# hardcamls/video-coding

Measured on AMD Instinct MI355X. Metric: Mpixel/s decoded (1080p 4:2:0 batch), higher is better.
Workload: dtype int32

## Files before the change

### video-coding_amd/csrc/hvc_capi.hip

```cpp
#include <cmath>

#include "hvc_ctx.h"
#include "hvc_dct_fixed.h"

bool pin_to_ctx_cpus(const hvc_ctx *c) {
    if (!c->have_cpus) {
        if (c->have_default_cpus) (void)pthread_setaffinity_np(pthread_self(), sizeof(cpu_set_t), &c->default_cpus);
        return true;
    }
    return pthread_setaffinity_np(pthread_self(), sizeof(cpu_set_t), &c->cpus) == 0;
}

bool parse_cpulist(const char *s, cpu_set_t &set) {
    CPU_ZERO(&set);
    int n = 0;
    while (*s) {
        while (*s == ' ' || *s == '\n') s++;
        if (!*s) break;
        char *end = nullptr;
        const long a = std::strtol(s, &end, 10);
        if (end == s || a < 0) return false;
        long b = a;
        s = end;
        if (*s == '-') {
// ... 435 lines not shown
    c->profiling = enabled != 0;
    c->k_calls = 0;
    return HVC_OK;
} HVC_ABI_CATCH

int hvc_kernel_ms_history(hvc_ctx *c, float *ms, int n) try {
    if (!c || !ms || n < 1 || n > HVC_PROF_RING || (unsigned long long)n > c->k_calls) return HVC_E_INVALID_ARG;
    DeviceGuard g(c->device);
    for (int i = 0; i < n; i++) {
        int slot = (int)((c->k_calls - (unsigned long long)n + (unsigned long long)i) % HVC_PROF_RING);
        HIPCHK(c, hipEventSynchronize(c->k1[slot]));
        HIPCHK(c, hipEventElapsedTime(&ms[i], c->k0[slot], c->k1[slot]));
    }
    return HVC_OK;
} HVC_ABI_CATCH

int hvc_last_kernel_ms(hvc_ctx *c, float *ms) { return hvc_kernel_ms_history(c, ms, 1); }

int hvc_device_alloc(hvc_ctx *c, size_t bytes, void **out) try {
    if (!c || !out) return HVC_E_INVALID_ARG;
    DeviceGuard g(c->device);
    hipError_t e = hipMalloc(out, bytes ? bytes : 1);
    if (e != hipSuccess) {
        c->last_hip = (int)e;
        *out = nullptr;
        return HVC_E_OUT_OF_MEMORY;
    }
    return HVC_OK;
} HVC_ABI_CATCH

int hvc_device_free(hvc_ctx *c, void *p) try {
    if (!c) return HVC_E_INVALID_ARG;
    DeviceGuard g(c->device);
    HIPCHK(c, hipFree(p));
    return HVC_OK;
} HVC_ABI_CATCH

int hvc_memcpy_h2d(hvc_ctx *c, void *dst, const void *src, size_t bytes) try {
    if (!c || (!dst && bytes) || (!src && bytes)) return HVC_E_INVALID_ARG;
    DeviceGuard g(c->device);
    HIPCHK(c, hipMemcpyAsync(dst, src, bytes, hipMemcpyHostToDevice, c->stream));
    HIPCHK(c, hipStreamSynchronize(c->stream));
    return HVC_OK;
} HVC_ABI_CATCH

int hvc_memcpy_d2h(hvc_ctx *c, void *dst, const void *src, size_t bytes) try {
    if (!c || (!dst && bytes) || (!src && bytes)) return HVC_E_INVALID_ARG;
    DeviceGuard g(c->device);
    HIPCHK(c, hipMemcpyAsync(dst, src, bytes, hipMemcpyDeviceToHost, c->stream));
    HIPCHK(c, hipStreamSynchronize(c->stream));
    return HVC_OK;
} HVC_ABI_CATCH

int hvc_checksum_records(hvc_ctx *c, const void *data, size_t record_bytes, size_t record_stride, int n_records,
                         uint64_t *sums, int where) try {
    if (!c || !sums || n_records < 0 || (!data && n_records && record_bytes)) return HVC_E_INVALID_ARG;
    if (where != HVC_MEM_HOST && where != HVC_MEM_DEVICE) return HVC_E_INVALID_ARG;
    if (n_records == 0) return HVC_OK;
    if (n_records > 1 && record_stride < record_bytes) return HVC_E_INVALID_ARG;
    DeviceGuard g(c->device);
    if (!g.ok) return fail_hip(c, hipErrorInvalidDevice);
    const size_t sum_bytes = (size_t)n_records * sizeof(unsigned long long);
    const uint8_t *d = (const uint8_t *)data;
    int r;
    if (where == HVC_MEM_HOST) {
        const size_t bytes = (size_t)(n_records - 1) * record_stride + record_bytes;
        if ((r = grow(c, &c->d_in, &c->in_cap, bytes ? bytes : 1))) return r;
        if (bytes) HIPCHK(c, hipMemcpyAsync(c->d_in, data, bytes, hipMemcpyHostToDevice, c->stream));
        d = (const uint8_t *)c->d_in;
    }
    if ((r = grow(c, &c->d_sums, &c->sums_cap, sum_bytes))) return r;
    for (int r0 = 0; r0 < n_records; r0 += 65535)
        HIPCHK(c, hvc::launch_checksum(d + (size_t)r0 * record_stride, record_bytes, record_stride,
                                       n_records - r0 < 65535 ? n_records - r0 : 65535, (unsigned long long *)c->d_sums + r0, c->stream));
    HIPCHK(c, hipMemcpyAsync(sums, c->d_sums, sum_bytes, hipMemcpyDeviceToHost, c->stream));
    HIPCHK(c, hipStreamSynchronize(c->stream));
    return HVC_OK;
} HVC_ABI_CATCH

int hvc_last_wide_blocks(hvc_ctx *c, uint64_t *count) try {
    if (!c || !count) return HVC_E_INVALID_ARG;
    DeviceGuard g(c->device);
    unsigned long long v = 0;
    HIPCHK(c, hipMemcpyAsync(&v, c->d_fix_count + 2, sizeof v, hipMemcpyDeviceToHost, c->stream));
    HIPCHK(c, hipStreamSynchronize(c->stream));
    *count = c->wide_host >= 0 ? (uint64_t)c->wide_host : (uint64_t)v;
    return HVC_OK;
} HVC_ABI_CATCH

static void prepare_tables(const uint16_t *qtabs, int n_qtabs, int *qt, int *ethr, int *ethr_packed, unsigned *qpair) {
    for (int i = 0; i < n_qtabs * 64; i++) qt[i] = (int)qtabs[i];
    for (int t = 0; t < n_qtabs; t++) {
        unsigned qmax = 1;
        for (int i = 0; i < 64; i++) qmax = qtabs[t * 64 + i] > qmax ? qtabs[t * 64 + i] : qmax;
        unsigned long long m = HVC_GUARD_D / qmax;
        unsigned long long thr = m * m;
        ethr[t] = thr > 0x7ffffffeull ? 0x7ffffffe : (int)thr;
        m = HVC_GUARD_D_PACKED / qmax;
        thr = m * m;
        ethr_packed[t] = thr > 0x7ffffffeull ? 0x7ffffffe : (int)thr;
        static const int PAIRS[4][2] = {{HVC_PAIR_A_LO, HVC_PAIR_A_HI}, {HVC_PAIR_B_LO, HVC_PAIR_B_HI},
                                        {HVC_PAIR_C_LO, HVC_PAIR_C_HI}, {HVC_PAIR_Z_LO, HVC_PAIR_Z_HI}};
        for (int r = 0; r < 8; r++)
            for (int k = 0; k < 4; k++) {
                unsigned lo = qtabs[t * 64 + hvc::HVC_ZF[8 * r + PAIRS[k][0]]];
                unsigned hi = qtabs[t * 64 + hvc::HVC_ZF[8 * r + PAIRS[k][1]]];
                qpair[t * 32 + r * 4 + k] = (lo & 0xffffu) | (hi << 16);
            }
    }
}

static int upload_dcfix(hvc_ctx *c, const std::vector<unsigned> &ids, const std::vector<long long> &dcs, const unsigned **d_count,
                        const unsigned **d_ids, const long long **d_dcs) {
    const size_t n = ids.size();
    const size_t off_ids = 16, off_dcs = (off_ids + n * sizeof(unsigned) + 15) & ~(size_t)15;
    int r = grow(c, &c->d_dcfix, &c->dcfix_cap, off_dcs + n * sizeof(long long));
    if (r) return r;
    const unsigned cnt = (unsigned)n;
    char *base = (char *)c->d_dcfix;
    HIPCHK(c, hipMemcpyAsync(base, &cnt, sizeof cnt, hipMemcpyHostToDevice, c->stream));
    HIPCHK(c, hipMemcpyAsync(base + off_ids, ids.data(), n * sizeof(unsigned), hipMemcpyHostToDevice, c->stream));
    HIPCHK(c, hipMemcpyAsync(base + off_dcs, dcs.data(), n * sizeof(long long), hipMemcpyHostToDevice, c->stream));
    HIPCHK(c, hipStreamSynchronize(c->stream));
    *d_count = (const unsigned *)base;
    *d_ids = (const unsigned *)(base + off_ids);
    *d_dcs = (const long long *)(base + off_dcs);
    return HVC_OK;
}

template <class Params, class Geometry>
static void fill_geometry(Params &P, const Geometry &G, size_t coef_fs, size_t pixel_fs, int n_frames) {
    std::memset(&P, 0, sizeof P);
    P.coef_fs = coef_fs;
    P.pixel_fs = pixel_fs;
    P.n_frames = n_frames;
    P.n_comp = G.n_comp;
    P.tiles_per_frame = G.tiles_per_frame;
    for (int i = 0; i < G.n_comp; i++) P.comp[i] = G.comp[i];
}

static hvc::HardcamlParams hardcaml_params(const hvc::DecodeParams &P, const uint16_t *qtabs, int n_qtabs) {
    hvc::HardcamlParams H;
    fill_geometry(H, P, P.coef_fs, P.pixel_fs, P.n_frames);
    H.coefs = P.coefs;
    H.pixels = P.pixels;
    hvc::prepare_hardcaml_tables(qtabs, n_qtabs, H.qq);
    H.dc_plane = P.dc_plane;
    H.dc_fs = P.dc_fs;
    return H;
}

static int apply_wide_dc(hvc_ctx *c, const hvc::DecodeParams &P, const std::vector<WideFix> &wide, const uint16_t *qtabs,
                         int n_qtabs, int arith) {
    std::vector<unsigned> ids;
    std::vector<long long> dcs;
    for (const WideFix &w : wide) {
        for (int i = 0; i < P.n_comp; i++) {
            const hvc::CompK &K = P.comp[i];
            const size_t b0 = K.coef_off / 64;
            if (w.block < b0 || w.block >= b0 + (size_t)K.nblk) continue;
            const unsigned b = (unsigned)(w.block - b0);
            ids.push_back(((unsigned)w.frame * (unsigned)P.tiles_per_frame + (unsigned)K.tile0 + b / HVC_TILE) * HVC_TILE + b % HVC_TILE);
            dcs.push_back(w.dc);
            break;
        }
    }
    if (ids.empty()) return HVC_OK;
// ... 124 lines not shown

static int frames_per_launch_capped(int n_frames, unsigned long long blocks_per_frame, unsigned long long ids_per_frame) {
    int per = frames_per_launch(n_frames, blocks_per_frame);
    if (per > 65535) per = 65535;
    const unsigned long long by_ids = ids_per_frame ? ((1ull << 32) - 1) / ids_per_frame : (unsigned long long)per;
    if ((unsigned long long)per > by_ids) per = (int)by_ids;
    return per < 1 ? 1 : per;
}


static int reserve_fix_list(hvc_ctx *c, size_t entries) {
    if (entries <= c->fix_cap) return HVC_OK;
    void *p = c->d_fix_list;
    size_t cap = c->fix_cap * sizeof(unsigned);
    const int r = grow(c, &p, &cap, entries * sizeof(unsigned));
    c->d_fix_list = (unsigned *)p;
    c->fix_cap = cap / sizeof(unsigned);
    return r;
}

template <class Launch>
static hipError_t for_each_launch(int f0, int cnt, int per, hipEvent_t k0, hipEvent_t k1, Launch launch) {
    for (int f = f0; f < f0 + cnt; f += per) {
        const hipError_t e = launch(f, std::min(per, f0 + cnt - f), f == f0 ? k0 : nullptr, f + per >= f0 + cnt ? k1 : nullptr);
        if (e != hipSuccess) return e;
    }
    return hipSuccess;
}

template <class Up, class Run, class Down>
static int through_device(hvc_ctx *c, int n_frames, size_t in_bytes, size_t out_bytes, size_t coef_bytes, bool may_overlap, Up up, Run run,
                          Down down) {
    int r = grow(c, &c->d_in, &c->in_cap, in_bytes);
    if (r) return r;
    if ((r = grow(c, &c->d_out, &c->out_cap, out_bytes))) return r;
    if (may_overlap && n_frames >= 8 && coef_bytes >= ((size_t)64 << 20))
        return overlapped_parts(c, n_frames, up, [&](int, int f0, int cnt) { return run(f0, cnt); }, down);
    HIPCHK(c, up(0, n_frames));
    HIPCHK(c, run(0, n_frames));
    HIPCHK(c, down(0, n_frames, c->stream));
    HIPCHK(c, hipStreamSynchronize(c->stream));
    return HVC_OK;
}

static size_t tight_records(const hvc_component *comps, int n_comp, bool pixels, hvc_component *tight, int *blk0 = nullptr) {
    size_t at = 0;
    for (int i = 0; i < n_comp; i++) {
        tight[i] = comps[i];
        if (pixels) {
            tight[i].stride = (size_t)comps[i].blocks_w * 8;
            tight[i].plane_offset = at;
        } else {
            tight[i].coef_offset = at;
        }
        if (blk0) blk0[i] = (int)(at / 64);
        at += (size_t)comps[i].blocks_w * comps[i].blocks_h * 64;
    }
    return at;
}

int decode_frames_impl(hvc_ctx *c, const int16_t *coefs, size_t coef_fs, const uint16_t *qtabs, int n_qtabs,
                       const hvc_component *comps_in, int n_comp_in, int n_frames, uint8_t *pixels, size_t pixel_fs, int where,
                       const DecodeOpts &o) {
    if (!c || n_frames < 0) return HVC_E_INVALID_ARG;
    if (where != HVC_MEM_HOST && where != HVC_MEM_DEVICE) return HVC_E_INVALID_ARG;
    int r = check_qtabs(qtabs, n_qtabs, false);
    if (r) return r;
    hvc_component kept[HVC_MAX_COMP];
    int n_comp = 0;
    if ((r = drop_empty_components(comps_in, n_comp_in, kept, &n_comp))) return r;
    if (n_comp == 0) return HVC_OK;
    const hvc_component *const comps = kept;
    if (!coefs || !pixels) return HVC_E_INVALID_ARG;
    Layout L;
    r = make_layout(comps, n_comp, n_qtabs, L);
    if (r) return r;
    if (n_frames == 0) return HVC_OK;
    if (n_frames > 1 && (coef_fs < L.coef_span || pixel_fs < L.pixel_span)) return HVC_E_INVALID_ARG;
    if ((coef_fs & 7) || (pixel_fs & 7)) return HVC_E_ALIGNMENT;
    const unsigned long long ids_per_frame = (unsigned long long)L.tiles_per_frame * HVC_TILE;
    const int per = frames_per_launch_capped(n_frames, L.blocks_per_frame, ids_per_frame);
    const bool has_wide = o.wide && !o.wide->empty();
    if (has_wide && (unsigned long long)n_frames * ids_per_frame >= (1ull << 32)) return HVC_E_TOO_LARGE;
    DeviceGuard g(c->device);
    if (!g.ok) return fail_hip(c, hipErrorInvalidDevice);

    const bool twin = o.arith == HVC_ARITH_HARDCAML;
    if ((r = reserve_fix_list(c, twin ? 0 : (size_t)((unsigned long long)per * ids_per_frame)))) return r;

    hvc::DecodeParams P;
    fill_geometry(P, L, coef_fs, pixel_fs, n_frames);
    prepare_tables(qtabs, n_qtabs, P.qt, P.ethr, P.ethr_packed, P.qpair);
    wide_total_begin(c);
    fix_assign(c, P);

    bool wide_only = false;
    for (int i = 0; i < n_qtabs * 64; i++) wide_only |= qtabs[i] > 255;
    wide_only |= c->decode_kernel == 2;
    P.kernel_sel = (c->decode_kernel == 1 || c->decode_kernel == 3) ? c->decode_kernel : 0;
    if (wide_only) c->wide_host = (long long)((unsigned long long)n_frames * L.blocks_per_frame);
    if (twin) c->wide_host = 0;
    auto launch = [&](hvc::DecodeParams &Q, hipEvent_t k0, hipEvent_t k1) -> hipError_t {
        if (twin) return hvc::launch_hardcaml(hardcaml_params(Q, qtabs, n_qtabs), c->stream, k0, k1);
        if (wide_only) return hvc::launch_decode_wide_only(Q, c->stream, k0, k1);
        fix_assign(c, Q);
        const hipError_t e = hvc::launch_decode(Q, c->stream, k0, k1);
        if (e == hipSuccess) fix_commit(c);
        else fix_reset(c);
        return e;
    };
    auto launch_range = [&](const int16_t *d_coefs, uint8_t *d_pixels, int f0, int cnt, hipEvent_t k0, hipEvent_t k1) {
        return for_each_launch(f0, cnt, per, k0, k1, [&](int f, int n, hipEvent_t e0, hipEvent_t e1) {
            hvc::DecodeParams Pk = P;
            Pk.n_frames = n;
            Pk.coefs = d_coefs + (size_t)f * coef_fs;
            Pk.pixels = d_pixels + (size_t)f * pixel_fs;
            if (o.dc_plane) Pk.dc_plane = o.dc_plane + (size_t)f * o.dc_fs;
            return launch(Pk, e0, e1);
        });
    };

    if (where == HVC_MEM_DEVICE) {
        if (((uintptr_t)coefs & 15) || ((uintptr_t)pixels & 7)) return HVC_E_ALIGNMENT;
        if (o.dc_plane && P.kernel_sel != 0 && !twin) return HVC_E_INVALID_ARG;
        P.coefs = coefs;
        P.pixels = pixels;
        P.dc_plane = o.dc_plane;
        P.dc_fs = o.dc_fs;
        const int slot = (int)(c->k_calls % HVC_PROF_RING);
        HIPCHK(c, launch_range(coefs, pixels, 0, n_frames, o.profile ? c->k0[slot] : nullptr, o.profile ? c->k1[slot] : nullptr));
        if (o.profile) c->k_calls++;
        if (has_wide) return apply_wide_dc(c, P, *o.wide, qtabs, n_qtabs, o.arith);
        return HVC_OK;
    }
    if (o.dc_plane || has_wide) return HVC_E_INVALID_ARG;

    const size_t cbytes = ((size_t)(n_frames - 1) * coef_fs + L.coef_span) * sizeof(int16_t);
    const size_t pbytes = (size_t)(n_frames - 1) * pixel_fs + L.pixel_span;
    const RecordRun run = pixel_run(comps, n_comp);
    return through_device(
        c, n_frames, cbytes, pbytes, cbytes, run.len != 0,
        [&](int f0, int cnt) {
            return hipMemcpyAsync((int16_t *)c->d_in + (size_t)f0 * coef_fs, coefs + (size_t)f0 * coef_fs,
                                  ((size_t)(cnt - 1) * coef_fs + L.coef_span) * sizeof(int16_t), hipMemcpyHostToDevice, c->stream);
        },
        [&](int f0, int cnt) { return launch_range((const int16_t *)c->d_in, (uint8_t *)c->d_out, f0, cnt, nullptr, nullptr); },
        [&](int f0, int cnt, hipStream_t st) {
            return download_pixels(comps, n_comp, run, f0, cnt, pixel_fs, (const uint8_t *)c->d_out, pixels, st);
        });
}

int hvc_decode_frames(hvc_ctx *c, const int16_t *coefs, size_t coef_fs, const uint16_t *qtabs, int n_qtabs,
                      const hvc_component *comps, int n_comp, int n_frames, uint8_t *pixels, size_t pixel_fs,
                      int where) try {
    return decode_frames_impl(c, coefs, coef_fs, qtabs, n_qtabs, comps, n_comp, n_frames, pixels, pixel_fs, where, DecodeOpts(c));
} HVC_ABI_CATCH

int hvc_decode_frames_mixed(hvc_ctx *c, const int16_t *coefs, const size_t *coef_offsets, const hvc_jpeg_info *infos, int n_frames,
                            uint8_t *pixels, const size_t *pixel_offsets, int where) try {
    return decode_frames_mixed_impl(c, coefs, coef_offsets, infos, n_frames, pixels, pixel_offsets, where);
} HVC_ABI_CATCH

int decode_frames_scaled_impl(hvc_ctx *c, const int16_t *coefs, size_t coef_fs, const uint16_t *qtabs, int n_qtabs,
                              const hvc_component *comps_in, int n_comp_in, int n_frames, int scale_denom, uint8_t *pixels,
                              size_t pixel_fs, int where, const DecodeOpts &o) {
    const int N = scaled_side(scale_denom);
    if (!c || !N) return HVC_E_INVALID_ARG;
    if (N == 8) return decode_frames_impl(c, coefs, coef_fs, qtabs, n_qtabs, comps_in, n_comp_in, n_frames, pixels, pixel_fs, where, o);
    if (o.arith != HVC_ARITH_MODEL) return HVC_E_INVALID_ARG;
    if (n_frames < 0 || (where != HVC_MEM_HOST && where != HVC_MEM_DEVICE)) return HVC_E_INVALID_ARG;
    int r = check_qtabs(qtabs, n_qtabs, false);
    if (r) return r;
    hvc_component kept[HVC_MAX_COMP];
    int n_comp = 0;
    if ((r = drop_empty_components(comps_in, n_comp_in, kept, &n_comp))) return r;
    if (n_comp == 0) return HVC_OK;
    const hvc_component *const comps = kept;
    if (!coefs || !pixels) return HVC_E_INVALID_ARG;
    Layout L;
    if ((r = make_layout(comps, n_comp, n_qtabs, L, N))) return r;
    if (n_frames == 0) return HVC_OK;
    if (n_frames > 1 && (coef_fs < L.coef_span || pixel_fs < L.pixel_span)) return HVC_E_INVALID_ARG;
    if (coef_fs & 7) return HVC_E_ALIGNMENT;
    const int per = frames_per_launch_capped(n_frames, L.blocks_per_frame, (unsigned long long)L.tiles_per_frame * HVC_TILE);
    DeviceGuard g(c->device);
    if (!g.ok) return fail_hip(c, hipErrorInvalidDevice);

    hvc::DecodeParams P;
    fill_geometry(P, L, coef_fs, pixel_fs, n_frames);
    for (int i = 0; i < n_qtabs * 64; i++) P.qt[i] = (int)qtabs[i];
    P.wide_total = reinterpret_cast<unsigned long long *>(c->d_fix_count + 2);
    wide_total_begin(c);
    bool rows_on_dwords = ((n_frames > 1 ? pixel_fs : 0) & 3) == 0;
    for (int i = 0; i < n_comp; i++) rows_on_dwords &= ((comps[i].plane_offset | comps[i].stride) & 3) == 0;

    auto launch_range = [&](const int16_t *d_coefs, uint8_t *d_pixels, int f0, int cnt, hipEvent_t k0, hipEvent_t k1) {
        const bool dwords = rows_on_dwords && ((uintptr_t)d_pixels & 3) == 0;
        return for_each_launch(f0, cnt, per, k0, k1, [&](int f, int n, hipEvent_t e0, hipEvent_t e1) {
            hvc::DecodeParams Pk = P;
            Pk.n_frames = n;
            Pk.coefs = d_coefs + (size_t)f * coef_fs;
            Pk.pixels = d_pixels + (size_t)f * pixel_fs;
            Pk.dc_plane = o.dc_plane ? o.dc_plane + (size_t)f * o.dc_fs : nullptr;
            Pk.dc_fs = o.dc_fs;
            return hvc::launch_decode_scaled(Pk, N, dwords, c->stream, e0, e1);
        });
    };

    if (where == HVC_MEM_DEVICE) {
        if ((uintptr_t)coefs & 15) return HVC_E_ALIGNMENT;
        HIPCHK(c, hipMemsetAsync(P.wide_total, 0, sizeof *P.wide_total, c->stream));
        const int slot = (int)(c->k_calls % HVC_PROF_RING);
        HIPCHK(c, launch_range(coefs, pixels, 0, n_frames, o.profile ? c->k0[slot] : nullptr, o.profile ? c->k1[slot] : nullptr));
        if (o.profile) c->k_calls++;
        return HVC_OK;
    }
    if (o.dc_plane) return HVC_E_INVALID_ARG;

    const size_t cbytes = ((size_t)(n_frames - 1) * coef_fs + L.coef_span) * sizeof(int16_t);
    const size_t pbytes = (size_t)(n_frames - 1) * pixel_fs + L.pixel_span;
    return through_device(
        c, n_frames, cbytes, pbytes, cbytes, false,
        [&](int f0, int cnt) {
            const hipError_t e = hipMemsetAsync(P.wide_total, 0, sizeof *P.wide_total, c->stream);
            if (e != hipSuccess) return e;
            return hipMemcpyAsync((int16_t *)c->d_in + (size_t)f0 * coef_fs, coefs + (size_t)f0 * coef_fs,
                                  ((size_t)(cnt - 1) * coef_fs + L.coef_span) * sizeof(int16_t), hipMemcpyHostToDevice, c->stream);
        },
        [&](int f0, int cnt) { return launch_range((const int16_t *)c->d_in, (uint8_t *)c->d_out, f0, cnt, nullptr, nullptr); },
        [&](int f0, int cnt, hipStream_t st) {
            for (int f = f0; f < f0 + cnt; f++)
                for (int i = 0; i < n_comp; i++) {
                    const hvc_component &k = comps[i];
                    const size_t off = (size_t)f * pixel_fs + k.plane_offset;
                    const hipError_t e = hipMemcpy2DAsync(pixels + off, k.stride, (const uint8_t *)c->d_out + off, k.stride,
                                                          (size_t)k.blocks_w * N, (size_t)k.blocks_h * N, hipMemcpyDeviceToHost, st);
                    if (e != hipSuccess) return e;
                }
            return hipSuccess;
        });
}

int hvc_decode_frames_scaled(hvc_ctx *c, const int16_t *coefs, size_t coef_fs, const uint16_t *qtabs, int n_qtabs,
                             const hvc_component *comps, int n_comp, int n_frames, int scale_denom, uint8_t *pixels, size_t pixel_fs,
                             int where) try {
    return decode_frames_scaled_impl(c, coefs, coef_fs, qtabs, n_qtabs, comps, n_comp, n_frames, scale_denom, pixels, pixel_fs, where,
                                     DecodeOpts(c));
} HVC_ABI_CATCH

int hvc_decode_frames_rgb(hvc_ctx *c, const int16_t *coefs, size_t coef_fs, const uint16_t *qtabs, int n_qtabs, const hvc_component *comps,
                          int n_comp, int sampling, int n_frames, int width, int height, uint8_t *rgb, size_t rgb_row_stride,
                          size_t rgb_frame_stride, int layout, int where) try {
    RgbImage im;
    bool nothing = false;
    if (!coefs || !qtabs || !comps || !rgb) return HVC_E_INVALID_ARG;
    int r = rgb_check_args(c, sampling, width, height, n_frames, layout, where, rgb_row_stride, rgb_frame_stride, im, nothing);
    if (r) return r;
    if (n_comp != (sampling == HVC_YUV_400 ? 1 : 3)) return HVC_E_INVALID_ARG;
    if ((r = check_qtabs(qtabs, n_qtabs, false))) return r;
    if (nothing) return HVC_OK;
    int cw, ch;
    rgb_chroma_window(sampling, width, height, cw, ch);
    size_t coef_span = 0;
    for (int k = 0; k < n_comp; k++) {
        if (comps[k].blocks_w < 1 || comps[k].blocks_h < 1) return HVC_E_INVALID_ARG;
        if ((k ? cw : width) > 8 * comps[k].blocks_w || (k ? ch : height) > 8 * comps[k].blocks_h) return HVC_E_INVALID_ARG;
        coef_span = std::max(coef_span, comps[k].coef_offset + (size_t)comps[k].blocks_w * comps[k].blocks_h * 64);
    }
    hvc_component tight[HVC_MAX_COMP];
    const size_t px_fs = tight_records(comps, n_comp, true, tight);
    if (n_frames > 1 && coef_fs < coef_span) return HVC_E_INVALID_ARG;
    if (coef_fs & 7) return HVC_E_ALIGNMENT;
    if (where == HVC_MEM_DEVICE && ((uintptr_t)coefs & 15)) return HVC_E_ALIGNMENT;
    DeviceGuard g(c->device);
// ... 68 lines not shown
    int blk0[HVC_MAX_COMP];
    const size_t px_fs = tight_records(kept, n_comp, true, tight, blk0), blocks = px_fs / 64;
    Layout L;
    if ((r = make_layout(tight, n_comp, n_qtabs, L))) return r;
    if (n_frames > 1 && (coef_fs < L.coef_span || diff_fs < blocks)) return HVC_E_INVALID_ARG;
    if (coef_fs & 7) return HVC_E_ALIGNMENT;
    if (where == HVC_MEM_DEVICE && ((uintptr_t)coefs & 15)) return HVC_E_ALIGNMENT;
    DeviceGuard g(c->device);
    if (!g.ok) return fail_hip(c, hipErrorInvalidDevice);
    DecodeOpts model(c);
    model.arith = HVC_ARITH_MODEL;
    model.profile = false;
    return divergence_chunks(
        c, (const uint8_t *)coefs, coef_fs * sizeof(int16_t), L.coef_span * sizeof(int16_t), px_fs, n_frames, max_diff, diff_fs, blocks, where,
        [&](const uint8_t *d_in, int cnt) {
            return decode_frames_impl(c, (const int16_t *)d_in, coef_fs, qtabs, n_qtabs, tight, n_comp, cnt, (uint8_t *)c->d_div_px, px_fs,
                                      HVC_MEM_DEVICE, model);
        },
        [&](const uint8_t *d_in, int cnt, uint8_t *d_diff) {
            hvc::DecodeParams P;
            fill_geometry(P, L, coef_fs, px_fs, cnt);
            P.coefs = (const int16_t *)d_in;
            P.pixels = (uint8_t *)c->d_div_px;
            hvc::HardcamlParams H = hardcaml_params(P, qtabs, n_qtabs);
            H.diff = d_diff;
            H.diff_fs = diff_fs;
            for (int i = 0; i < n_comp; i++) H.blk0[i] = blk0[i];
            return hvc::launch_hardcaml(H, c->stream);
        });
} HVC_ABI_CATCH

int decode_frames_yuv444_impl(hvc_ctx *c, const int16_t *coefs, size_t coef_fs, const uint16_t *qtabs, int n_qtabs,
                              const hvc_component *comps, int n_comp, int n_frames, int width, int height, uint8_t *frames,
                              size_t frame_stride, int where, const DecodeOpts &o) {
    if (!c || !coefs || !frames || !comps || n_frames < 0) return HVC_E_INVALID_ARG;
    if (o.arith != HVC_ARITH_MODEL) return HVC_E_INVALID_ARG;
    if (where != HVC_MEM_HOST && where != HVC_MEM_DEVICE) return HVC_E_INVALID_ARG;
    int r = check_qtabs(qtabs, n_qtabs, false);
    if (r) return r;
    if (n_comp != 3 || width < 2 || height < 2 || (width & 1) || (height & 1)) return HVC_E_INVALID_ARG;
    if (width > 65535 || height > 65535) return HVC_E_TOO_LARGE;
    Layout L;
    hvc_component geo[3];
    for (int i = 0; i < 3; i++) {
        geo[i] = comps[i];
        geo[i].plane_offset = 0;
        geo[i].stride = comps[i].blocks_w > 0 ? (size_t)comps[i].blocks_w * 8 : 0;
    }
    r = make_layout(geo, n_comp, n_qtabs, L);
    if (r) return r;
    const int aw[3] = {width, width / 2, width / 2}, ah[3] = {height, height / 2, height / 2};
    for (int i = 0; i < 3; i++)
        if (comps[i].blocks_w * 8 < aw[i] || comps[i].blocks_h * 8 < ah[i]) return HVC_E_INVALID_ARG;
    const size_t plane_bytes = (size_t)width * (size_t)height, out_span = 3 * plane_bytes;
    if (n_frames == 0) return HVC_OK;
    if (n_frames > 1 && (coef_fs < L.coef_span || frame_stride < out_span)) return HVC_E_INVALID_ARG;
    if (coef_fs & 7) return HVC_E_ALIGNMENT;

    hvc::Decode444Params P;
    std::memset(&P, 0, sizeof P);
    P.coef_fs = coef_fs;
    P.out_fs = frame_stride;
    P.n_frames = n_frames;
    P.width = width;
    P.height = height;
    for (int i = 0; i < 3; i++) {
        hvc::Plane444K &K = P.pl[i];
        K.bw = comps[i].blocks_w;
        K.cbw = (aw[i] + 7) / 8;
        K.cbh = (ah[i] + 7) / 8;
        K.aw = aw[i];
        K.ah = ah[i];
        K.qtab = comps[i].qtab;
        K.coef_off = comps[i].coef_offset;
        K.out_off = (size_t)i * plane_bytes;
    }
    if ((unsigned long long)P.pl[0].cbw * P.pl[0].cbw * P.pl[0].cbh >= (1ull << 32)) return HVC_E_TOO_LARGE;
    const bool aligned = width % 16 == 0 && frame_stride % 16 == 0 && (where == HVC_MEM_HOST || (uintptr_t)frames % 16 == 0);
    hvc::plan_decode_444(P, aligned);
    const unsigned long long ids_per_frame = (unsigned long long)P.tiles_per_frame * HVC_TILE * P.nw;
    const int per = frames_per_launch_capped(n_frames, L.blocks_per_frame, ids_per_frame);
    const bool has_wide = o.wide && !o.wide->empty();
    if (has_wide && (unsigned long long)n_frames * ids_per_frame >= (1ull << 32)) return HVC_E_TOO_LARGE;
    const unsigned long long ids = (unsigned long long)per * ids_per_frame;
    DeviceGuard g(c->device);
    if (!g.ok) return fail_hip(c, hipErrorInvalidDevice);
    int ethr_unused[HVC_MAX_QTABS];
    prepare_tables(qtabs, n_qtabs, P.qt, ethr_unused, P.ethr_packed, P.qpair);
    bool wide_only = c->decode_kernel == 2;
    for (int i = 0; i < n_qtabs * 64; i++) wide_only |= qtabs[i] > 255;
    const int split = (aligned && !wide_only && c->decode_kernel == 0 && height % 8 == 0 && P.pl[0].cbw == P.pl[0].bw) ? fused444_mode() : 0;
    const size_t luma_ids = split ? (size_t)per * (size_t)((P.pl[0].cbw * P.pl[0].cbh + HVC_TILE - 1) / HVC_TILE) * HVC_TILE : 0;
    if ((r = reserve_fix_list(c, luma_ids + (size_t)ids))) return r;
    P.fix_list = c->d_fix_list;
    wide_total_begin(c);
    if (split == 2 && !c->side_stream) {
        static const int prio_sel = [] { const char *v = std::getenv("HVC_444_SIDE_PRIO"); return v ? std::atoi(v) : 0; }();
        int least = 0, greatest = 0;
        HIPCHK(c, hipDeviceGetStreamPriorityRange(&least, &greatest));
        HIPCHK(c, hipStreamCreateWithPriority(&c->side_stream, hipStreamNonBlocking, prio_sel < 0 ? greatest : prio_sel > 0 ? least : 0));
        HIPCHK(c, hipEventCreateWithFlags(&c->ev_fork, hipEventDisableTiming));
        HIPCHK(c, hipEventCreateWithFlags(&c->ev_join, hipEventDisableTiming));
    }
    auto launch_split = [&](hvc::Decode444Params &Q, hipEvent_t k0, hipEvent_t k1) -> hipError_t {
        const hvc::Plane444K &K = Q.pl[0];
        hvc::DecodeParams Y;
        std::memset(&Y, 0, sizeof Y);
        Y.coefs = Q.coefs;
        Y.pixels = Q.out;
        Y.coef_fs = Q.coef_fs;
        Y.pixel_fs = Q.out_fs;
        Y.n_frames = Q.n_frames;
        Y.n_comp = 1;
        Y.comp[0].bw = K.cbw;
        Y.comp[0].bh = K.cbh;
        Y.comp[0].nblk = K.cbw * K.cbh;
        Y.comp[0].magic = K.cbw == 1 ? 0u : (unsigned)(((1ull << 32) + (unsigned)K.cbw - 1) / (unsigned)K.cbw);
        Y.comp[0].qtab = K.qtab;
        Y.comp[0].coef_off = K.coef_off;
        Y.comp[0].plane_off = K.out_off;
        Y.comp[0].stride = (size_t)Q.width;
        Y.tiles_per_frame = (Y.comp[0].nblk + HVC_TILE - 1) / HVC_TILE;
        prepare_tables(qtabs, n_qtabs, Y.qt, Y.ethr, Y.ethr_packed, Y.qpair);
        Y.dc_plane = Q.dc_plane;
        Y.dc_fs = Q.dc_fs;
        Y.fix_count = c->d_fix_count + 4 + c->fix_phase_l;
        Y.fix_count_next = c->d_fix_count + 4 + (c->fix_phase_l ^ 1);
        Y.fix_list = c->d_fix_list + (size_t)ids;
        Y.wide_total = reinterpret_cast<unsigned long long *>(c->d_fix_count + 2);
        fix_assign(c, Q);
        Q.tile0 = Q.y_tiles;
        hipStream_t ys = c->stream;
        hipError_t e = hipSuccess;
        if (k0) e = hipEventRecord(k0, c->stream);
        if (split == 2) {
            if (e == hipSuccess && !c->wide_total_started) e = hipMemsetAsync(Y.wide_total, 0, sizeof(unsigned long long), c->stream);
            Y.wide_first = Q.wide_first = 2;
            if (e == hipSuccess) e = hipEventRecord(c->ev_fork, c->stream);
            if (e == hipSuccess) e = hipStreamWaitEvent(c->side_stream, c->ev_fork, 0);
            ys = c->side_stream;
        } else {
            Y.wide_first = Q.wide_first;
            Q.wide_first = 0;
        }
        if (e == hipSuccess) e = hvc::launch_decode(Y, ys, nullptr, nullptr);
        if (e == hipSuccess) c->fix_phase_l ^= 1;
        if (e == hipSuccess) e = hvc::launch_decode_444(Q, false, c->stream, nullptr, nullptr);
        if (e == hipSuccess && split == 2) {
            e = hipEventRecord(c->ev_join, c->side_stream);
            if (e == hipSuccess) e = hipStreamWaitEvent(c->stream, c->ev_join, 0);
        }
        if (e == hipSuccess && k1) e = hipEventRecord(k1, c->stream);
        if (e == hipSuccess) fix_commit(c);
        else {
            if (c->side_stream) (void)hipStreamSynchronize(c->side_stream);
            fix_reset(c);
        }
        return e;
    };
    auto launch = [&](hvc::Decode444Params &Q, hipEvent_t k0, hipEvent_t k1) -> hipError_t {
        if (wide_only) {
            c->wide_host = (long long)n_frames * ((long long)P.pl[0].cbw * P.pl[0].cbh + 2ll * P.pl[1].cbw * P.pl[1].cbh);
            return hvc::launch_decode_444(Q, true, c->stream, k0, k1);
        }
        if (split) return launch_split(Q, k0, k1);
        fix_assign(c, Q);
        const hipError_t e = hvc::launch_decode_444(Q, false, c->stream, k0, k1);
        if (e == hipSuccess) fix_commit(c);
        else fix_reset(c);
        return e;
    };

    auto launch_range = [&](const int16_t *d_coefs, uint8_t *d_out, int f0, int cnt, hipEvent_t k0, hipEvent_t k1) {
        return for_each_launch(f0, cnt, per, k0, k1, [&](int f, int n, hipEvent_t e0, hipEvent_t e1) {
            hvc::Decode444Params Pk = P;
            Pk.n_frames = n;
            Pk.coefs = d_coefs + (size_t)f * coef_fs;
            Pk.out = d_out + (size_t)f * frame_stride;
            if (o.dc_plane) Pk.dc_plane = o.dc_plane + (size_t)f * o.dc_fs;
            return launch(Pk, e0, e1);
        });
    };

    if (where == HVC_MEM_HOST && (o.dc_plane || has_wide)) return HVC_E_INVALID_ARG;
    if (where == HVC_MEM_DEVICE) {
        if ((uintptr_t)coefs & 15) return HVC_E_ALIGNMENT;
        P.coefs = coefs;
        P.out = frames;
        P.dc_plane = o.dc_plane;
        P.dc_fs = o.dc_fs;
        const bool prof = o.profile && !wide_only;
        const int slot = (int)(c->k_calls % HVC_PROF_RING);
        HIPCHK(c, launch_range(coefs, frames, 0, n_frames, prof ? c->k0[slot] : nullptr, prof ? c->k1[slot] : nullptr));
        if (prof) c->k_calls++;
        if (has_wide) return apply_wide_dc_444(c, P, *o.wide);
        return HVC_OK;
    }
    const size_t cbytes = ((size_t)(n_frames - 1) * coef_fs + L.coef_span) * sizeof(int16_t);
    const size_t obytes = (size_t)(n_frames - 1) * frame_stride + out_span;
    return through_device(
        c, n_frames, cbytes, obytes, cbytes, true,
        [&](int f0, int cnt) {
            return hipMemcpyAsync((int16_t *)c->d_in + (size_t)f0 * coef_fs, coefs + (size_t)f0 * coef_fs,
                                  ((size_t)(cnt - 1) * coef_fs + L.coef_span) * sizeof(int16_t), hipMemcpyHostToDevice, c->stream);
        },
        [&](int f0, int cnt) { return launch_range((const int16_t *)c->d_in, (uint8_t *)c->d_out, f0, cnt, nullptr, nullptr); },
        [&](int f0, int cnt, hipStream_t st) {
            return copy_run_d2h((const uint8_t *)c->d_out, frames, 0, out_span, frame_stride, f0, cnt, st);
        });
}

int hvc_decode_frames_yuv444(hvc_ctx *c, const int16_t *coefs, size_t coef_fs, const uint16_t *qtabs, int n_qtabs,
// ... 470 lines not shown
```

### video-coding_amd/csrc/hvc_capi_mixed.hip

```cpp
#include "hvc_ctx.h"
#include "hvc_mixed.h"

namespace {

struct ImageParts {
    size_t planes = 0, tables = 0, map = 0, total = 0;
};
ImageParts image_parts(const hvc::MixedPlan &plan) {
    ImageParts p;
    auto up = [](size_t v) { return (v + 15) & ~(size_t)15; };
    p.planes = 0;
    p.tables = up(plan.planes.size() * sizeof(hvc::MixedPlaneK));
    p.map = p.tables + up(plan.tables.size() * sizeof(hvc::MixedTableK));
    p.total = p.map + up(plan.map.size() * sizeof(unsigned));
    return p;
}

int upload_plan(hvc_ctx *c, const hvc::MixedPlan &plan, hvc::MixedParams &P) {
    const ImageParts ip = image_parts(plan);
    std::vector<unsigned char> img(ip.total, 0);
    std::memcpy(img.data() + ip.planes, plan.planes.data(), plan.planes.size() * sizeof(hvc::MixedPlaneK));
    std::memcpy(img.data() + ip.tables, plan.tables.data(), plan.tables.size() * sizeof(hvc::MixedTableK));
    std::memcpy(img.data() + ip.map, plan.map.data(), plan.map.size() * sizeof(unsigned));
    if (!c->ev_mixed) HIPCHK(c, hipEventCreateWithFlags(&c->ev_mixed, hipEventDisableTiming));
    const bool same = c->mixed_len == ip.total && c->h_mixed && !std::memcmp(c->h_mixed, img.data(), ip.total);
    if (!same) {
        c->mixed_len = 0;
        int r = grow(c, &c->d_mixed, &c->mixed_cap, ip.total);
        if (r) return r;
        if (ip.total > c->h_mixed_cap) {
            HIPCHK(c, hipStreamSynchronize(c->stream));
            if (c->h_mixed) (void)hipHostFree(c->h_mixed);
            c->h_mixed = nullptr;
            c->h_mixed_cap = 0;
            const size_t want = ip.total + ip.total / 4 + 4096;
            if (hipHostMalloc(&c->h_mixed, want, hipHostMallocDefault) != hipSuccess) {
                c->h_mixed = nullptr;
                return HVC_E_OUT_OF_MEMORY;
            }
            c->h_mixed_cap = want;
        } else {
            HIPCHK(c, wait_event(c->ev_mixed));
        }
        std::memcpy(c->h_mixed, img.data(), ip.total);
        HIPCHK(c, hipMemcpyAsync(c->d_mixed, c->h_mixed, ip.total, hipMemcpyHostToDevice, c->stream));
        HIPCHK(c, hipEventRecord(c->ev_mixed, c->stream));
        c->mixed_len = ip.total;
    }
    const unsigned char *d = (const unsigned char *)c->d_mixed;
    P.planes = reinterpret_cast<const hvc::MixedPlaneK *>(d + ip.planes);
    P.tables = reinterpret_cast<const hvc::MixedTableK *>(d + ip.tables);
    P.map = reinterpret_cast<const unsigned *>(d + ip.map);
    P.n_units = (unsigned)plan.map.size();
    return HVC_OK;
}

int reserve_mixed_fix_list(hvc_ctx *c, size_t entries) {
    if (entries <= c->fix_cap) return HVC_OK;
    void *p = c->d_fix_list;
    size_t cap = c->fix_cap * sizeof(unsigned);
    const int r = grow(c, &p, &cap, entries * sizeof(unsigned));
    c->d_fix_list = (unsigned *)p;
    c->fix_cap = cap / sizeof(unsigned);
    return r;
}

int mixed_launch_plan(hvc_ctx *c, const hvc::MixedPlan &plan, const int16_t *d_coefs, uint8_t *d_pixels, bool profile) {
    int r;
    if (plan.map.empty()) return HVC_OK;
    if (((uintptr_t)d_coefs & 15) || ((uintptr_t)d_pixels & 7)) return HVC_E_ALIGNMENT;
    if ((r = reserve_mixed_fix_list(c, plan.map.size() * HVC_MIXED_UNIT))) return r;
    hvc::MixedParams P;
    std::memset(&P, 0, sizeof P);
    if ((r = upload_plan(c, plan, P))) return r;
    P.coefs = d_coefs;
    P.pixels = d_pixels;
    P.all_wide = c->decode_kernel == 2;
    fix_assign(c, P);
    const int slot = (int)(c->k_calls % HVC_PROF_RING);
    const hipError_t e = hvc::launch_decode_mixed(P, c->stream, profile ? c->k0[slot] : nullptr, profile ? c->k1[slot] : nullptr);
    if (e != hipSuccess) {
        fix_reset(c);
        return fail_hip(c, e);
    }
    fix_commit(c);
    if (profile) c->k_calls++;
    return HVC_OK;
}

int mixed_launch(hvc_ctx *c, const int16_t *d_coefs, const size_t *coef_offsets, const hvc_jpeg_info *infos, const int *frames,
                 int n_list, uint8_t *d_pixels, const size_t *pixel_offsets, bool profile) {
    hvc::MixedPlan plan;
    const int r = hvc::mixed_plan_build(infos, coef_offsets, pixel_offsets, frames, n_list, plan);
    return r ? r : mixed_launch_plan(c, plan, d_coefs, d_pixels, profile);
}

void frame_spans(const hvc_jpeg_info &fi, size_t &coef_span, size_t &pixel_span) {
    coef_span = pixel_span = 0;
    for (int i = 0; i < fi.n_comp && i < 4; i++) {
        const hvc_component &k = fi.layout[i];
        if (k.blocks_w <= 0 || k.blocks_h <= 0) continue;
        coef_span = std::max(coef_span, k.coef_offset + (size_t)k.blocks_w * k.blocks_h * 64);
        pixel_span = std::max(pixel_span, k.plane_offset + ((size_t)k.blocks_h * 8 - 1) * k.stride + (size_t)k.blocks_w * 8);
    }
}

}

int decode_frames_mixed_impl(hvc_ctx *c, const int16_t *coefs, const size_t *coef_offsets, const hvc_jpeg_info *infos, int n_frames,
                             uint8_t *pixels, const size_t *pixel_offsets, int where) {
    if (!c || n_frames < 0 || (where != HVC_MEM_HOST && where != HVC_MEM_DEVICE)) return HVC_E_INVALID_ARG;
    if (c->arith != HVC_ARITH_MODEL) return HVC_E_INVALID_ARG;
    if (n_frames == 0) return HVC_OK;
    if (!infos || !coef_offsets || !pixel_offsets) return HVC_E_INVALID_ARG;
    DeviceGuard g(c->device);
    if (!g.ok) return fail_hip(c, hipErrorInvalidDevice);
    int r;
    {
        hvc::MixedPlan plan;
        if ((r = hvc::mixed_plan_build(infos, coef_offsets, pixel_offsets, nullptr, n_frames, plan))) return r;
        if (plan.map.empty()) return HVC_OK;
        if (!coefs || !pixels) return HVC_E_INVALID_ARG;
        if (where == HVC_MEM_DEVICE) {
            wide_total_begin(c);
            return mixed_launch_plan(c, plan, coefs, pixels, c->profiling);
        }
    }
    std::vector<size_t> d_coef((size_t)n_frames), d_pix((size_t)n_frames), cspan((size_t)n_frames);
    size_t ctot = 0, ptot = 0;
    for (int f = 0; f < n_frames; f++) {
        size_t ps;
        frame_spans(infos[f], cspan[(size_t)f], ps);
        d_coef[(size_t)f] = ctot;
        d_pix[(size_t)f] = ptot;
        ctot += (cspan[(size_t)f] + 63) & ~(size_t)63;
        ptot += (ps + 63) & ~(size_t)63;
    }
    if ((r = grow(c, &c->d_in, &c->in_cap, ctot * sizeof(int16_t)))) return r;
    if ((r = grow(c, &c->d_out, &c->out_cap, ptot))) return r;
    for (int f = 0; f < n_frames; f++)
        if (cspan[(size_t)f])
            HIPCHK(c, hipMemcpyAsync((int16_t *)c->d_in + d_coef[(size_t)f], coefs + coef_offsets[f], cspan[(size_t)f] * sizeof(int16_t),
                                     hipMemcpyHostToDevice, c->stream));
    wide_total_begin(c);
    if ((r = mixed_launch(c, (const int16_t *)c->d_in, d_coef.data(), infos, nullptr, n_frames, (uint8_t *)c->d_out, d_pix.data(), false))) {
        (void)hipStreamSynchronize(c->stream);
        return r;
    }
    for (int f = 0; f < n_frames; f++)
        for (int i = 0; i < infos[f].n_comp; i++) {
            const hvc_component &k = infos[f].layout[i];
            if (k.blocks_w <= 0 || k.blocks_h <= 0) continue;
            const size_t row = (size_t)k.blocks_w * 8, rows = (size_t)k.blocks_h * 8;
            uint8_t *dst = pixels + pixel_offsets[f] + k.plane_offset;
// ... 269 lines not shown
```

### video-coding_amd/csrc/hvc_ctx.h

```cpp
#ifndef HVC_CTX_H
#define HVC_CTX_H

#include <hip/hip_runtime.h>
#include <pthread.h>
#include <sched.h>

#include <algorithm>
#include <atomic>
#include <chrono>
#include <condition_variable>
#include <cstdio>
#include <cstdlib>
#include <cstring>
#include <mutex>
#include <new>
#include <thread>
#include <deque>
#include <functional>
#include <vector>

#include "../../include/hvc_jpeg.h"
#include "hvc_hdec.h"
#include "hvc_hardcaml.h"
#include "hvc_huff.h"
#include "hvc_kernels.h"
#include "hvc_pool.h"
#include "hvc_scaled_spec.h"

#define HVC_PROF_RING 64
#define HVC_FIX_WORDS 8

struct hvc_ctx {
    int device = -1;
    hipStream_t own_stream = nullptr;
    hipStream_t stream = nullptr;
    hipEvent_t ev0 = nullptr, ev1 = nullptr;
    hipEvent_t k0[HVC_PROF_RING] = {}, k1[HVC_PROF_RING] = {};
    unsigned long long k_calls = 0;
    bool profiling = false;
    bool honour_restart = false;
    int decode_kernel = 0;
    int arith = HVC_ARITH_MODEL;
    int enc_arith = HVC_ARITH_MODEL;
    int huff_tables = HVC_HUFF_DEFAULT;
    int restart_interval = 0;
    unsigned *d_fix_count = nullptr;
    int fix_phase_l = 0;
    hipStream_t side_stream = nullptr;
    hipEvent_t ev_fork = nullptr, ev_join = nullptr;
    bool wide_total_started = false;
    long long wide_host = -1;
    int fix_phase = 0;
    int fix_last = 0;
    unsigned *d_fix_list = nullptr;
    size_t fix_cap = 0;
    void *d_in = nullptr, *d_out = nullptr, *d_sums = nullptr, *d_aux = nullptr, *d_aux2 = nullptr;
    size_t in_cap = 0, out_cap = 0, sums_cap = 0, aux_cap = 0, aux2_cap = 0;
    void *d_div_px = nullptr, *d_div_in = nullptr, *d_div_out = nullptr;
    size_t div_px_cap = 0, div_in_cap = 0, div_out_cap = 0;
    void *d_dct_tab = nullptr, *d_dct_a = nullptr, *d_dct_b = nullptr;
    size_t dct_a_cap = 0, dct_b_cap = 0;
    int last_hip = 0;
    static constexpr int RING = 3;
    hipStream_t copy_stream = nullptr, down_stream = nullptr;
    hipStream_t rd_stream[3] = {};
    hipEvent_t ev_rd[3] = {};
    void *h_ring[RING] = {}, *d_ring[RING] = {}, *d_oring[RING] = {};
    size_t ring_bytes = 0, oring_bytes = 0;
    hipEvent_t ev_h2d[RING] = {}, ev_kern[RING] = {}, ev_t[4] = {};
    void *eh_in[RING] = {}, *ed_in[RING] = {}, *eh_out[RING] = {}, *ed_out[RING] = {};
    size_t e_in_bytes = 0, e_out_bytes = 0;
    hipEvent_t ev_up[RING] = {}, ev_down[RING] = {}, ev_et[RING][3] = {}, ev_gpu[RING] = {};
    void *ed_seg[RING] = {}, *ed_off[RING] = {}, *eh_off[RING] = {};
    size_t e_seg_bytes = 0, e_off_bytes = 0;
    void *eh_specs[RING] = {};
    size_t e_specs_bytes = 0;
    void *gp_h_ecs[RING] = {}, *gp_d_ecs[RING] = {}, *gp_h_meta[RING] = {}, *gp_d_meta[RING] = {};
    void *gp_h_ftabs[RING] = {}, *gp_d_ftabs[RING] = {};
    size_t gp_ecs_bytes = 0, gp_meta_bytes = 0, gp_ftabs_bytes = 0;
    void *gd_ecs = nullptr, *gd_meta = nullptr, *gd_state = nullptr, *gd_tables = nullptr, *gd_coefs = nullptr, *gd_dcd = nullptr;
    void *gd_h_ecs = nullptr;
    size_t gd_h_ecs_cap = 0;
    void *gd_fcnt = nullptr;
    size_t gd_fcnt_cap = 0;
    void *gd_ftabs = nullptr;
    size_t gd_ftabs_cap = 0;
    void *gd_dcv = nullptr;
    size_t gd_dcv_cap = 0;
    void *d_dcfix = nullptr;
    size_t dcfix_cap = 0;
    void *d_mixed = nullptr, *h_mixed = nullptr;
    size_t mixed_cap = 0, h_mixed_cap = 0, mixed_len = 0;
    hipEvent_t ev_mixed = nullptr;
    bool have_cpus = false;
    cpu_set_t cpus;
    char cpulist[256] = "";
    bool have_default_cpus = false;
    cpu_set_t default_cpus;
    hvc::WorkerPool pool;
    hvc::HdTables *gd_tables_host = nullptr;
    bool gd_tables_valid = false;
    int gd_tables_ncomp = 0;
    size_t gd_ecs_cap = 0, gd_meta_cap = 0, gd_state_cap = 0, gd_tables_cap = 0, gd_coefs_cap = 0, gd_dcd_cap = 0;
    unsigned *hd_tables = nullptr;
    void *hd_opt = nullptr;
    size_t hd_opt_cap = 0;
    void *hd_lens = nullptr, *hd_meta = nullptr, *hd_bitbuf = nullptr, *hd_ff = nullptr, *hd_out = nullptr;
    size_t hd_lens_cap = 0, hd_meta_cap = 0, hd_bitbuf_cap = 0, hd_ff_cap = 0, hd_out_cap = 0;
    void *hd_ivl = nullptr;
    size_t hd_ivl_cap = 0;
    struct Slot {
        void *d_in = nullptr, *d_out = nullptr;
        size_t in_cap = 0, out_cap = 0;
        hipEvent_t up0 = nullptr, up1 = nullptr, k0 = nullptr, k1 = nullptr, dn0 = nullptr, dn1 = nullptr;
        bool busy = false, has_down = false, timed = false;
        unsigned long long h2d_bytes = 0, d2h_bytes = 0;
    } slots[HVC_SLOTS];
};

#ifndef HVC_UPLOAD_RING_FLAGS
#define HVC_UPLOAD_RING_FLAGS hipHostMallocDefault
#endif

struct DeviceGuard {
    int prev = -1;
    bool ok = true;
    explicit DeviceGuard(int dev) {
        if (hipGetDevice(&prev) != hipSuccess) prev = -1;
        if (prev != dev) ok = hipSetDevice(dev) == hipSuccess;
    }
    ~DeviceGuard() {
        int cur = -1;
        if (prev >= 0 && hipGetDevice(&cur) == hipSuccess && cur != prev) (void)hipSetDevice(prev);
    }
};

inline int fail_hip(hvc_ctx *c, hipError_t e) {
    c->last_hip = (int)e;
    return HVC_E_HIP;
}
#define HIPCHK(c, call)                                 \
    do {                                                \
        hipError_t e_ = (call);                         \
        if (e_ != hipSuccess) return fail_hip((c), e_); \
    } while (0)

bool pin_to_ctx_cpus(const hvc_ctx *c);

inline int pool_ready(hvc_ctx *c, int n, int extra = 0) { return c->pool.ensure(n + extra); }

bool parse_cpulist(const char *s, cpu_set_t &set);

int grow(hvc_ctx *c, void **p, size_t *cap, size_t need);

template <class Params>
inline void fix_assign(const hvc_ctx *c, Params &P) {
    P.fix_count = c->d_fix_count + c->fix_phase;
    P.fix_count_next = c->d_fix_count + (c->fix_phase ^ 1);
    P.fix_list = c->d_fix_list;
    P.wide_total = reinterpret_cast<unsigned long long *>(c->d_fix_count + 2);
    P.wide_first = c->wide_total_started ? 0 : 1;
}
inline void fix_commit(hvc_ctx *c) {
    c->fix_last = c->fix_phase;
    c->fix_phase ^= 1;
    c->wide_total_started = true;
}
inline void wide_total_begin(hvc_ctx *c) {
    c->wide_total_started = false;
    c->wide_host = -1;
}
inline void fix_reset(hvc_ctx *c) {
    (void)hipMemsetAsync(c->d_fix_count, 0, HVC_FIX_WORDS * sizeof(unsigned), c->stream);
}

size_t launch_bytes_limit();
#ifndef HVC_444_MODE_DEFAULT
#define HVC_444_MODE_DEFAULT 0
#endif
int fused444_mode();
int frames_per_launch(int n_frames, unsigned long long blocks_per_frame);

struct Layout {
    hvc::CompK comp[HVC_MAX_COMP];
    int n_comp = 0, tiles_per_frame = 0;
    size_t coef_span = 0;
    size_t pixel_span = 0;
    unsigned long long blocks_per_frame = 0;
};
int make_layout(const hvc_component *comps, int n_comp, int n_qtabs, Layout &L, int n = 8);
int check_qtabs(const uint16_t *qtabs, int n_qtabs, bool divides);

int drop_empty_components(const hvc_component *comps, int n_comp, hvc_component *kept, int *n_kept);

struct RecordRun {
    size_t first = 0, len = 0;
};
RecordRun pixel_run(const hvc_component *comps, int n_comp);
RecordRun coef_run(const hvc_component *comps, int n_comp);
hipError_t download_pixels(const hvc_component *comps, int n_comp, const RecordRun &run, int f0, int cnt, size_t fs,
                           const uint8_t *d_base, uint8_t *h_base, hipStream_t st);
hipError_t download_coefs(const hvc_component *comps, int n_comp, const RecordRun &run, int f0, int cnt, size_t fs_bytes,
                          const uint8_t *d_base, uint8_t *h_base, hipStream_t st);

hipError_t wait_event(hipEvent_t e);

template <class Up, class Run, class Down>
inline int overlapped_parts(hvc_ctx *c, int n_frames, Up up, Run run, Down down) {
    constexpr int K = 4;
    if (!c->down_stream) HIPCHK(c, hipStreamCreateWithFlags(&c->down_stream, hipStreamNonBlocking));
    for (int i = 0; i < K; i++)
        if (!c->ev_t[i]) HIPCHK(c, hipEventCreate(&c->ev_t[i]));
    std::atomic<int> launched{0}, herr{0};
    auto part = [&](int k, int &f0, int &cnt) {
        f0 = (int)((long long)n_frames * k / K);
        cnt = (int)((long long)n_frames * (k + 1) / K) - f0;
    };
    int pr = pool_ready(c, 1);
    if (pr) return pr;
    hvc::PoolScope scope(c->pool, [&] { if (launched.load() < K) herr.store(herr.load() ? herr.load() : (int)hipErrorUnknown); });
    pr = c->pool.submit([&] {
        (void)pin_to_ctx_cpus(c);
        if (hipSetDevice(c->device) != hipSuccess) { herr.store((int)hipErrorInvalidDevice); return; }
        for (int k = 0; k < K; k++) {
            while (launched.load(std::memory_order_acquire) <= k && !herr.load()) std::this_thread::yield();
            if (herr.load()) return;
            int f0, cnt;
            part(k, f0, cnt);
            hipError_t e = hipStreamWaitEvent(c->down_stream, c->ev_t[k], 0);
            if (e == hipSuccess) e = down(f0, cnt, c->down_stream);
            if (e == hipSuccess) e = hipStreamSynchronize(c->down_stream);
            if (e != hipSuccess) { herr.store((int)e); return; }
        }
    }, 1);
    if (pr) return pr;
    hipError_t e = hipSuccess;
    for (int k = 0; k < K && e == hipSuccess && !herr.load(); k++) {
        int f0, cnt;
        part(k, f0, cnt);
        e = up(f0, cnt);
        if (e == hipSuccess) e = run(k, f0, cnt);
        if (e == hipSuccess) e = hipEventRecord(c->ev_t[k], c->stream);
        if (e == hipSuccess) launched.store(k + 1, std::memory_order_release);
// ... 132 lines not shown
```

### video-coding_amd/csrc/hvc_kernels.h

```cpp
#ifndef HVC_KERNELS_H
#define HVC_KERNELS_H

#include <hip/hip_runtime.h>
#include <cstdlib>
#include <stddef.h>
#include <stdint.h>

#define HVC_MAX_COMP 4
#define HVC_MAX_QTABS 4
#define HVC_GUARD_D ((1 << 17) - 1)
#define HVC_TILE 256

#include "hvc_idct_spec.h"

namespace hvc {

static const unsigned char HVC_ZF[64] = {
    0,  1,  5,  6,  14, 15, 27, 28, 2,  4,  7,  13, 16, 26, 29, 42, 3,  8,  12, 17, 25, 30,
    41, 43, 9,  11, 18, 24, 31, 40, 44, 53, 10, 19, 23, 32, 39, 45, 52, 54, 20, 22, 33, 38,
    46, 51, 55, 60, 21, 34, 37, 47, 50, 56, 59, 61, 35, 36, 48, 49, 57, 58, 62, 63};

struct CompK {
    int bw, bh;
    int nblk;
    int tile0;
    unsigned magic;
    int qtab;
    size_t coef_off;
    size_t plane_off;
    size_t stride;
};

struct DecodeParams {
    const int16_t *coefs;
    uint8_t *pixels;
    size_t coef_fs;
    size_t pixel_fs;
    int n_frames, n_comp, tiles_per_frame;
    int kernel_sel;
    CompK comp[HVC_MAX_COMP];
    int qt[HVC_MAX_QTABS * 64];
    int ethr[HVC_MAX_QTABS];
    unsigned qpair[HVC_MAX_QTABS * 32];
    int ethr_packed[HVC_MAX_QTABS];
    unsigned *fix_count;
    unsigned *fix_count_next;
    unsigned *fix_list;
    const int16_t *dc_plane;
    size_t dc_fs;
    unsigned long long *wide_total;
    int wide_first;
    int xcd_map;
    unsigned xcd_magic;
};

struct EncodeParams {
    const uint8_t *pixels;
    int16_t *coefs;
    size_t coef_fs, pixel_fs;
    int n_frames, n_comp, tiles_per_frame, xcd_map;
    unsigned xcd_magic, pad;
    CompK comp[HVC_MAX_COMP];
    float qrcp[HVC_MAX_QTABS * 64];
};

struct UpsampleParams {
    const uint8_t *src;
    uint8_t *dst;
    int cw, ch, n_planes, xcd_map;
    size_t src_stride, dst_stride, src_ps, dst_ps;
    unsigned xcd_magic, pad;
};

struct Plane444K {
    int bw;
    int cbw, cbh;
    int aw, ah;
    int qtab;
    size_t coef_off;
    size_t out_off;
};

#define HVC_444_TILE_BW 64
#define HVC_444_TILE_BH 4

struct Decode444Params {
    const int16_t *coefs;
    uint8_t *out;
    size_t coef_fs;
    size_t out_fs;
    int n_frames, tiles_per_frame;
    int width, height;
    int y_tiles;
    unsigned y_magic;
    int c_tiles_x, c_tiles_y;
    unsigned c_magic;
    int skip;
    int nw;
    int tile0;
    Plane444K pl[3];
    int qt[HVC_MAX_QTABS * 64];
    unsigned qpair[HVC_MAX_QTABS * 32];
    int ethr_packed[HVC_MAX_QTABS];
    unsigned *fix_count, *fix_count_next, *fix_list;
    const int16_t *dc_plane;
    size_t dc_fs;
    unsigned long long *wide_total;
    int wide_first;
    int xcd_map;
    unsigned xcd_magic;
};

inline int xcd_map_run(bool fused = false) {
    static const int run = [] { const char *v = getenv("HVC_XCD_RUN"); return v ? atoi(v) : -1; }();
    static const int run444 = [] { const char *v = getenv("HVC_XCD_RUN_444"); return v ? atoi(v) : -1; }();
    if (fused) return run444 >= 0 ? run444 : run >= 0 ? run : 64;
    return run >= 0 ? run : 16;
}
#ifdef __HIPCC__
__device__ __forceinline__ void xcd_work(int map, unsigned magic, unsigned &frame, unsigned &tile) {
    frame = blockIdx.y;
    tile = blockIdx.x;
    if (map > 0) {
        const unsigned per = gridDim.x, id = frame * per + tile, sh = (unsigned)map - 1u;
        const unsigned group = 8u << sh, total = per * gridDim.y;
        if (id < total - total % group) {
            const unsigned k = id >> 3;
            const unsigned lin = ((((k >> sh) << 3) + (id & 7u)) << sh) + (k & ((1u << sh) - 1u));
            frame = __umulhi(lin, magic);
            tile = lin - frame * per;
        }
    }
}
#endif
inline int xcd_map_for(unsigned per, unsigned n, unsigned &magic, bool fused = false) {
    magic = per > 1 ? (unsigned)(((1ull << 32) + per - 1) / per) : 0u;
    const int run = xcd_map_run(fused);
    if (run <= 0 || per <= 1 || (unsigned long long)per * n * per >= (1ull << 32)) return 0;
    int sh = 0;
    while ((1 << (sh + 1)) <= run) sh++;
    return sh + 1;
}

hipError_t launch_decode_444(const Decode444Params &P, bool wide_only, hipStream_t s, hipEvent_t k0 = nullptr,
                             hipEvent_t k1 = nullptr);
void plan_decode_444(Decode444Params &P, bool aligned);
hipError_t launch_decode(const DecodeParams &P, hipStream_t s, hipEvent_t k0 = nullptr, hipEvent_t k1 = nullptr);
hipError_t launch_decode_wide_only(const DecodeParams &P, hipStream_t s, hipEvent_t k0 = nullptr, hipEvent_t k1 = nullptr);
hipError_t launch_decode_dcfix(const DecodeParams &P, const unsigned *count, const unsigned *ids, const long long *dcs,
                               hipStream_t s);
hipError_t launch_decode_444_dcfix(const Decode444Params &P, const unsigned *count, const unsigned *ids, const long long *dcs,
                                   unsigned n_host, hipStream_t s);
hipError_t launch_encode(const EncodeParams &P, hipStream_t s, hipEvent_t k0 = nullptr, hipEvent_t k1 = nullptr);
hipError_t launch_upsample420(const UpsampleParams &P, hipStream_t s);
hipError_t launch_abs_error(const EncodeParams &P, const uint8_t *recon, uint8_t *error, hipStream_t s);
#define HVC_CHECKSUM_MUL 0x9E3779B97F4A7C15ull
hipError_t launch_checksum(const uint8_t *data, size_t record_bytes, size_t record_stride, int n_records,
                           unsigned long long *sums, hipStream_t s);

}
#endif
```

### video-coding_amd/csrc/hvc_kernels.hip

```cpp

#include <hip/hip_runtime.h>
#include <stdint.h>
#include <stdlib.h>
#include <string.h>

#include "hvc_idct_spec.h"
#include "hvc_kernels.h"

#ifndef HVC_FAST_LB
#define HVC_FAST_LB HVC_TILE
#endif

namespace hvc {

__device__ constexpr int ZI[64] = {
    0,  1,  8,  16, 9,  2,  3,  10, 17, 24, 32, 25, 18, 11, 4,  5,
    12, 19, 26, 33, 40, 48, 41, 34, 27, 20, 13, 6,  7,  14, 21, 28,
    35, 42, 49, 56, 57, 50, 43, 36, 29, 22, 15, 23, 30, 37, 44, 51,
    58, 59, 52, 45, 38, 31, 39, 46, 53, 60, 61, 54, 47, 55, 62, 63};
__device__ constexpr int ZF[64] = {
    0,  1,  5,  6,  14, 15, 27, 28, 2,  4,  7,  13, 16, 26, 29, 42,
    3,  8,  12, 17, 25, 30, 41, 43, 9,  11, 18, 24, 31, 40, 44, 53,
    10, 19, 23, 32, 39, 45, 52, 54, 20, 22, 33, 38, 46, 51, 55, 60,
    21, 34, 37, 47, 50, 56, 59, 61, 35, 36, 48, 49, 57, 58, 62, 63};
// ... 147 lines not shown
    size_t coef_idx;
    size_t pix_idx;
    size_t stride;
    int qtab;
    size_t plane_coef_idx;
    int tile_b0;
    int nblk;
};

template <class Params>
__device__ __forceinline__ bool locate(const Params &P, int frame, int tile, int lane, BlockRef &br) {
    int c = 0;
#pragma unroll
    for (int i = 1; i < HVC_MAX_COMP; i++)
        if (i < P.n_comp && tile >= P.comp[i].tile0) c = i;
    const CompK &K = P.comp[c];
    int b = (tile - K.tile0) * HVC_TILE + lane;
    bool active = b < K.nblk;
    b = active ? b : K.nblk - 1;
    unsigned by = K.bw == 1 ? (unsigned)b : __umulhi((unsigned)b, K.magic);
    unsigned bx = (unsigned)b - by * (unsigned)K.bw;
    br.coef_idx = (size_t)frame * P.coef_fs + K.coef_off + (size_t)b * 64;
    br.pix_idx = (size_t)frame * P.pixel_fs + K.plane_off + (size_t)by * 8 * K.stride + (size_t)bx * 8;
    br.stride = K.stride;
    br.qtab = K.qtab;
    br.plane_coef_idx = (size_t)frame * P.coef_fs + K.coef_off;
    br.tile_b0 = (tile - K.tile0) * HVC_TILE;
    br.nblk = K.nblk;
    return active;
}

__global__ __launch_bounds__(HVC_FAST_LB) void k_decode_fast(DecodeParams P) {
    BlockRef br;
    const int lane = threadIdx.x;
    const bool active = locate(P, blockIdx.y, blockIdx.x, lane, br);

    const uint4 *src = reinterpret_cast<const uint4 *>(P.coefs + br.coef_idx);
    uint4 raw[8];
#pragma unroll
    for (int j = 0; j < 8; j++) raw[j] = src[j];

    const int *__restrict__ q = P.qt + br.qtab * 64;

    int v[64];
    Guard g;
#pragma unroll
    for (int j = 0; j < 8; j++) {
        const unsigned w[4] = {raw[j].x, raw[j].y, raw[j].z, raw[j].w};
#pragma unroll
        for (int h = 0; h < 4; h++) {
            const int k = j * 8 + h * 2;
            g.e2(w[h]);
            v[ZI[k]] = dequant_lo(w[h], q[k]);
            v[ZI[k + 1]] = dequant_hi(w[h], q[k + 1]);
        }
    }

#pragma unroll
    for (int r = 0; r < 8; r++) {
        idct_1d_fast<false, 0>(v[r * 8 + 0], v[r * 8 + 1], v[r * 8 + 2], v[r * 8 + 3], v[r * 8 + 4],
                               v[r * 8 + 5], v[r * 8 + 6], v[r * 8 + 7], g);
        g.r2(v[r * 8 + 0], v[r * 8 + 1]);
        g.r2(v[r * 8 + 2], v[r * 8 + 3]);
        g.r2(v[r * 8 + 4], v[r * 8 + 5]);
        g.r2(v[r * 8 + 6], v[r * 8 + 7]);
    }
#pragma unroll
    for (int c = 0; c < 8; c++)
        idct_1d_fast<true, (128 << 14)>(v[c], v[8 + c], v[16 + c], v[24 + c], v[32 + c], v[40 + c],
                                        v[48 + c], v[56 + c], g);

    const bool bad = g.bad(P.ethr[br.qtab]);
    if (active && !bad) {
#pragma unroll
        for (int j = 0; j < 8; j++) {
            uint2 o;
            o.x = ashr14_sat_pack4(v[j * 8 + 0], v[j * 8 + 1], v[j * 8 + 2], v[j * 8 + 3]);
            o.y = ashr14_sat_pack4(v[j * 8 + 4], v[j * 8 + 5], v[j * 8 + 6], v[j * 8 + 7]);
            store_row8(P.pixels + br.pix_idx + (size_t)j * br.stride, o.x, o.y);
        }
    }
    const bool flag = active && bad;
    const unsigned long long m = __ballot(flag);
    if (m) {
        const int wl = lane & 63;
        unsigned base = 0;
        if (wl == 0) base = atomicAdd(P.fix_count, (unsigned)__popcll(m));
        base = __shfl(base, 0);
        if (flag) {
            unsigned idx = base + (unsigned)__popcll(m & ((1ull << wl) - 1ull));
            P.fix_list[idx] = ((unsigned)blockIdx.y * (unsigned)P.tiles_per_frame + blockIdx.x) * HVC_TILE + lane;
        }
    }
}

typedef short short2v __attribute__((ext_vector_type(2)));
typedef unsigned short ushort2v __attribute__((ext_vector_type(2)));

template <int ADD>
__device__ __forceinline__ int dot2(unsigned pair, unsigned k) {
    static_assert(ADD == 0 || ADD == 4, "inline constants only");
    int d;
    if (ADD == 0)
        asm("v_dot2_i32_i16 %0, %1, %2, 0" : "=v"(d) : "v"(pair), "s"(k));
    else
        asm("v_dot2_i32_i16 %0, %1, %2, 4" : "=v"(d) : "v"(pair), "s"(k));
    return d;
}
__device__ __forceinline__ int dot2v(unsigned pair, unsigned k, int add) {
    int d;
    asm("v_dot2_i32_i16 %0, %1, %2, %3" : "=v"(d) : "v"(pair), "s"(k), "v"(add));
    return d;
}
__device__ __forceinline__ int dot2_sat(unsigned pair, unsigned k, int acc) {
    return __builtin_amdgcn_sdot2(__builtin_bit_cast(short2v, pair), __builtin_bit_cast(short2v, k), acc, true);
}
constexpr unsigned pk(int lo, int hi) { return ((unsigned)lo & 0xffffu) | ((unsigned)hi << 16); }

template <int PA, int PB>
__device__ __forceinline__ unsigned gather_pair(const unsigned (&w)[32]) {
    constexpr int za = ZF[PA], zb = ZF[PB];
    constexpr int ha = za & 1, hb = zb & 1;
    constexpr unsigned sel = ((unsigned)(4 + 2 * hb + 1) << 24) | ((unsigned)(4 + 2 * hb) << 16) |
                             ((unsigned)(2 * ha + 1) << 8) | (unsigned)(2 * ha);
    return __builtin_amdgcn_perm(w[zb >> 1], w[za >> 1], sel);
}
__device__ __forceinline__ unsigned pk_mul_lo(unsigned a, unsigned b) {
    return __builtin_bit_cast(unsigned, (ushort2v)(__builtin_bit_cast(ushort2v, a) * __builtin_bit_cast(ushort2v, b)));
}

struct PackedGuard {
    int energy = 0;
    int renergy = 0;
    int ymax = 0, ymin = 0;
    int k128 = HVC_ROW_ZADD, kcol = HVC_COL_ZADD;
    __device__ __forceinline__ void y2(int a, int b) { ymax = max(max(ymax, a), b); ymin = min(min(ymin, a), b); }
};
constexpr int GUARD_RE = HVC_GUARD_RE;

#define HVC_EXPAND_PASS(PASS)                                                                                           \
    HVC_IDCT_PASS(HVC_OP_ROT_##PASS, HVC_OP_ZDOT_##PASS, HVC_OP_ADD, HVC_OP_SUB, HVC_OP_GUARDY, HVC_OP_M181,            \
                  HVC_OP_OUTADD_##PASS, HVC_OP_OUTSUB_##PASS)
#define HVC_OP_ROT_ROW(d, P, klo, khi) const int d = dot2<HVC_ROW_RADD>(P, pk(klo, khi)) >> HVC_ROW_RSHIFT;
#define HVC_OP_ROT_COL(d, P, klo, khi) const int d = dot2<HVC_COL_RADD>(P, pk(klo, khi)) >> HVC_COL_RSHIFT;
#define HVC_OP_ZDOT_ROW(d, P, slo, shi) const int d = dot2v(P, pk((slo) * HVC_ROW_ZSCALE, (shi) * HVC_ROW_ZSCALE), g.k128);
#define HVC_OP_ZDOT_COL(d, P, slo, shi) const int d = dot2v(P, pk((slo) * HVC_COL_ZSCALE, (shi) * HVC_COL_ZSCALE), g.kcol);
#define HVC_OP_ADD(d, a, b) const int d = a + b;
#define HVC_OP_SUB(d, a, b) const int d = a - b;
#define HVC_OP_GUARDY(a, b) g.y2(a, b);
#define HVC_OP_M181(d, a) const int d = mad24(HVC_M181_MUL, a, HVC_M181_ADD) >> HVC_M181_SHIFT;
#define HVC_OP_OUTADD_ROW(i, a, b) o[i] = (a + b) >> HVC_ROW_OSHIFT;
#define HVC_OP_OUTSUB_ROW(i, a, b) o[i] = (a - b) >> HVC_ROW_OSHIFT;
#define HVC_OP_OUTADD_COL(i, a, b) o[i] = (a + b) >> HVC_COL_OSHIFT;
#define HVC_OP_OUTSUB_COL(i, a, b) o[i] = (a - b) >> HVC_COL_OSHIFT;

template <int R>
__device__ __forceinline__ void idct_row_packed(const unsigned (&w)[32], const unsigned *__restrict__ qp, int (&o)[8],
                                                PackedGuard &g) {
    const unsigned A = pk_mul_lo(gather_pair<8 * R + HVC_PAIR_A_LO, 8 * R + HVC_PAIR_A_HI>(w), qp[0]);
    const unsigned B = pk_mul_lo(gather_pair<8 * R + HVC_PAIR_B_LO, 8 * R + HVC_PAIR_B_HI>(w), qp[1]);
    const unsigned C = pk_mul_lo(gather_pair<8 * R + HVC_PAIR_C_LO, 8 * R + HVC_PAIR_C_HI>(w), qp[2]);
    const unsigned Z = pk_mul_lo(gather_pair<8 * R + HVC_PAIR_Z_LO, 8 * R + HVC_PAIR_Z_HI>(w), qp[3]);
    HVC_EXPAND_PASS(ROW)
}

__device__ __forceinline__ unsigned pack_rows(int lo, int hi, PackedGuard &g) {
    const unsigned p = __builtin_bit_cast(unsigned, __builtin_amdgcn_cvt_pk_i16(lo, hi));
    g.renergy = dot2_sat(p, p, g.renergy);
    return p;
}

__device__ __forceinline__ void idct_col_packed(unsigned A, unsigned B, unsigned C, unsigned Z, int (&o)[8],
                                                PackedGuard &g) {
    HVC_EXPAND_PASS(COL)
}

// ... 32 lines not shown
        _Pragma("unroll") for (int j = 0; j < 8; j++) {                                                 \
            const uint4 t = HVC_PACKED_SRC(SRC, j);                                                     \
            w[4 * j + 0] = t.x;                                                                         \
            w[4 * j + 1] = t.y;                                                                         \
            w[4 * j + 2] = t.z;                                                                         \
            w[4 * j + 3] = t.w;                                                                         \
        }                                                                                               \
        PRE                                                                                             \
        HVC_TRAFFIC_ONLY_DECODE(OUT)                                                                    \
        _Pragma("unroll") for (int d = 0; d < 32; d++) (G).energy = dot2_sat(w[d], w[d], (G).energy);   \
                            \
        unsigned cA[8], cB[8], cC[8], cZ[8];                                                            \
        {                                                                                               \
            int ra[8], rb[8];                                                                           \
            idct_row_packed<HVC_PAIR_A_LO>(w, (QP) + 4 * HVC_PAIR_A_LO, ra, (G));                       \
            idct_row_packed<HVC_PAIR_A_HI>(w, (QP) + 4 * HVC_PAIR_A_HI, rb, (G));                       \
            _Pragma("unroll") for (int c = 0; c < 8; c++) cA[c] = pack_rows(ra[c], rb[c], (G));  \
            idct_row_packed<HVC_PAIR_B_LO>(w, (QP) + 4 * HVC_PAIR_B_LO, ra, (G));                       \
            idct_row_packed<HVC_PAIR_B_HI>(w, (QP) + 4 * HVC_PAIR_B_HI, rb, (G));                       \
            _Pragma("unroll") for (int c = 0; c < 8; c++) cB[c] = pack_rows(ra[c], rb[c], (G));  \
            idct_row_packed<HVC_PAIR_C_LO>(w, (QP) + 4 * HVC_PAIR_C_LO, ra, (G));                       \
            idct_row_packed<HVC_PAIR_C_HI>(w, (QP) + 4 * HVC_PAIR_C_HI, rb, (G));                       \
            _Pragma("unroll") for (int c = 0; c < 8; c++) cC[c] = pack_rows(ra[c], rb[c], (G));  \
            idct_row_packed<HVC_PAIR_Z_LO>(w, (QP) + 4 * HVC_PAIR_Z_LO, ra, (G));                       \
            idct_row_packed<HVC_PAIR_Z_HI>(w, (QP) + 4 * HVC_PAIR_Z_HI, rb, (G));                       \
            _Pragma("unroll") for (int c = 0; c < 8; c++) cZ[c] = pack_rows(ra[c], rb[c], (G));  \
        }                                                                                               \
                           \
        _Pragma("unroll") for (int c = 0; c < 8; c += 2) {                                              \
            int ca[8], cb[8];                                                                           \
            idct_col_packed(cA[c], cB[c], cC[c], cZ[c], ca, (G));                                       \
            idct_col_packed(cA[c + 1], cB[c + 1], cC[c + 1], cZ[c + 1], cb, (G));                       \
            _Pragma("unroll") for (int j = 0; j < 8; j++) {                                             \
                if ((c & 2) == 0)                                                                       \
                    ashr14_sat_pack2<0>((OUT)[j][c >> 2], ca[j], cb[j]);                                \
                else                                                                                    \
                    ashr14_sat_pack2<1>((OUT)[j][c >> 2], ca[j], cb[j]);                                \
            }                                                                                           \
        }                                                                                               \
    } while (0)

__device__ __forceinline__ bool packed_guard_failed(const PackedGuard &g, int ethr) {
    return (g.energy > ethr) | (g.renergy >= GUARD_RE) | (g.ymax > GUARD_Y) | (g.ymin < -GUARD_Y);
}

__device__ __forceinline__ unsigned with_dc(unsigned w0, int16_t dc) { return (w0 & 0xffff0000u) | (unsigned)(unsigned short)dc; }

template <bool DCP>
__global__ __launch_bounds__(HVC_PACKED_LB) void k_decode_packed(DecodeParams P) {
    BlockRef br;
    const int lane = threadIdx.x;
    unsigned wframe, wtile;
    xcd_work(P.xcd_map, P.xcd_magic, wframe, wtile);
    const bool active = locate(P, (int)wframe, (int)wtile, lane, br);
    const uint4 *src = reinterpret_cast<const uint4 *>(P.coefs + br.coef_idx);
    const unsigned *__restrict__ qp = P.qpair + br.qtab * 32;
    PackedGuard g;
    unsigned out[8][2];
    int16_t dcv = 0;
    if (DCP) dcv = P.dc_plane[(size_t)wframe * P.dc_fs + ((br.coef_idx - (size_t)wframe * P.coef_fs) >> 6)];
#if HVC_TRAFFIC_ONLY == 2
    const bool hvc_full = __ballot(active) == ~0ull;
    const int hvc_src_stride = hvc_full ? 64 : 1;
    if (hvc_full) src = src - 8 * (lane & 63) + (lane & 63);
#endif
    HVC_DECODE_BLOCK_PACKED(src, qp, out, g, if (DCP) w[0] = with_dc(w[0], dcv););
#ifdef HVC_K1_PAD_VALU
    {
        int pad = lane;
#pragma unroll
        for (int i = 0; i < HVC_K1_PAD_VALU; i++) asm volatile("v_mul_i32_i24 %0, %0, %1" : "+v"(pad) : "v"(lane));
        asm volatile("" ::"v"(pad));
    }
#endif

    const bool bad = packed_guard_failed(g, P.ethr_packed[br.qtab]);
    if (active && !bad) {
#pragma unroll
        for (int j = 0; j < 8; j++)
            store_row8(P.pixels + br.pix_idx + (size_t)j * br.stride, out[j][0], out[j][1]);
    }
    const bool flag = active && bad;
    const unsigned long long m = __ballot(flag);
    if (m) {
        const int wl = lane & 63;
        unsigned base = 0;
        if (wl == 0) base = atomicAdd(P.fix_count, (unsigned)__popcll(m));
        base = __shfl(base, 0);
        if (flag) {
            unsigned idx = base + (unsigned)__popcll(m & ((1ull << wl) - 1ull));
            P.fix_list[idx] = (wframe * (unsigned)P.tiles_per_frame + wtile) * HVC_TILE + lane;
        }
    }
}

constexpr int Q16_ITERS = HVC_TILE / 16;

__device__ __forceinline__ int dot2vv(unsigned pair, unsigned k, int add) {
    int d;
    asm("v_dot2_i32_i16 %0, %1, %2, %3" : "=v"(d) : "v"(pair), "v"(k), "v"(add));
    return d;
}
__device__ __forceinline__ int partner(int v) { return __builtin_amdgcn_mov_dpp(v, 0xB1, 0xf, 0xf, true); }

struct Q16Lane {
    unsigned k00, k01, k10, k11;
    int a0, a1, sh0, sh1;
};

__device__ __forceinline__ void q16_pass(unsigned P0, unsigned P1, const Q16Lane &K, bool odd, int negm, int (&o)[4],
                                         int &ymax, int &ymin) {
    const int p = dot2vv(P0, K.k00, K.a0) >> K.sh0, q = dot2vv(P0, K.k01, K.a0) >> K.sh0;
    const int s = dot2vv(P1, K.k10, K.a1) >> K.sh1, t = dot2vv(P1, K.k11, K.a1) >> K.sh1;
    const int u1 = p + s, u2 = p - s, u3 = q + t, u4 = q - t;
    const int ys = odd ? u2 + u4 : 0, yd = odd ? u2 - u4 : 0;
    ymax = max(max(ymax, ys), yd);
    ymin = min(min(ymin, ys), yd);
    const int w2 = mad24(181, ys, 128) >> 8, w4 = mad24(181, yd, 128) >> 8;
    const int m0 = u1, m1 = odd ? u3 : u2, m2 = odd ? w2 : u3, m3 = odd ? w4 : u4;
    o[0] = partner(m0) + ((m0 ^ negm) - negm);
    o[1] = partner(m1) + ((m1 ^ negm) - negm);
    o[2] = partner(m2) + ((m2 ^ negm) - negm);
    o[3] = partner(m3) + ((m3 ^ negm) - negm);
}

__global__ __launch_bounds__(HVC_TILE) void k_decode_q16(DecodeParams P) {
    __shared__ short stage[16][64];
    __shared__ uint8_t tile[8][HVC_TILE][8];
    __shared__ unsigned short qlds[64];
    __shared__ uint8_t badflag[HVC_TILE];

    const int lane = threadIdx.x, g = lane >> 4, l = lane & 15;
    BlockRef br;
    const bool active = locate(P, blockIdx.y, blockIdx.x, lane, br);
    if (lane < 64) qlds[lane] = (unsigned short)P.qt[br.qtab * 64 + lane];
    __syncthreads();

    const bool odd = l & 1;
    const int negm = odd ? -1 : 0;
    const int r = l >> 1;
    Q16Lane KR, KC;
    KR.k10 = odd ? pk(W5, W3) : pk(W2, W6);
    KR.k11 = odd ? pk(W3, -W5) : pk(W6, -W2);
    KR.k00 = odd ? pk(W1, W7) : pk(2048, 2048);
    KR.k01 = odd ? pk(W7, -W1) : pk(2048, -2048);
    KR.a0 = odd ? 0 : 128;
    KR.a1 = 0;
    KR.sh0 = KR.sh1 = 0;
    KC.k10 = KR.k10;
    KC.k11 = KR.k11;
    KC.k00 = odd ? pk(W1, W7) : pk(256, 256);
    KC.k01 = odd ? pk(W7, -W1) : pk(256, -256);
    KC.a0 = odd ? 4 : 8192 + (128 << 14);
    KC.a1 = 4;
    KC.sh0 = odd ? 3 : 0;
    KC.sh1 = 3;
    const unsigned q01 = qlds[4 * l] | ((unsigned)qlds[4 * l + 1] << 16), q23 = qlds[4 * l + 2] | ((unsigned)qlds[4 * l + 3] << 16);

    auto slot = [](int row, int col) {
        const int pos = (col & 1) ? ((col == 1) ? 0 : (col == 7) ? 1 : (col == 5) ? 2 : 3)
                                  : ((col == 0) ? 0 : (col == 4) ? 1 : (col == 2) ? 2 : 3);
        return (2 * row + (col & 1)) * 4 + pos;
    };
    int ld_slot[4];
#pragma unroll
    for (int i = 0; i < 4; i++) {
        const int p = ZI[4 * l + i];
        ld_slot[i] = slot(p >> 3, p & 7);
    }
    const int oc[4] = {odd ? 7 : 0, odd ? 4 : 3, odd ? 6 : 1, odd ? 5 : 2};
    int tr_slot[4];
#pragma unroll
    for (int i = 0; i < 4; i++) tr_slot[i] = slot(oc[i], r);

    const size_t plane_coefs = br.plane_coef_idx;
    for (int it = 0; it < Q16_ITERS; it++) {
        const int bi = it * 16 + g;
        int b = br.tile_b0 + bi;
        const bool exists = b < br.nblk;
        b = exists ? b : br.nblk - 1;
        const uint2 cz = reinterpret_cast<const uint2 *>(P.coefs + plane_coefs + (size_t)b * 64)[l];
        int energy = dot2_sat(cz.y, cz.y, dot2_sat(cz.x, cz.x, 0));
        const unsigned d01 = pk_mul_lo(cz.x, q01), d23 = pk_mul_lo(cz.y, q23);
        short *st = stage[g];
        st[ld_slot[0]] = (short)(d01 & 0xffffu);
        st[ld_slot[1]] = (short)(d01 >> 16);
        st[ld_slot[2]] = (short)(d23 & 0xffffu);
        st[ld_slot[3]] = (short)(d23 >> 16);
        __builtin_amdgcn_fence(__ATOMIC_RELEASE, "wavefront");
        __builtin_amdgcn_wave_barrier();
        __builtin_amdgcn_fence(__ATOMIC_ACQUIRE, "wavefront");
        uint2 ops = reinterpret_cast<const uint2 *>(st)[l];
        int ymax = 0, ymin = 0, o[4];
        q16_pass(ops.x, ops.y, KR, odd, negm, o, ymax, ymin);
        const unsigned r01 = __builtin_bit_cast(unsigned, __builtin_amdgcn_cvt_pk_i16(o[0] >> 8, o[1] >> 8));
        const unsigned r23 = __builtin_bit_cast(unsigned, __builtin_amdgcn_cvt_pk_i16(o[2] >> 8, o[3] >> 8));
        int renergy = dot2_sat(r23, r23, dot2_sat(r01, r01, 0));
        __builtin_amdgcn_fence(__ATOMIC_RELEASE, "wavefront");
        __builtin_amdgcn_wave_barrier();
        st[tr_slot[0]] = (short)(r01 & 0xffffu);
        st[tr_slot[1]] = (short)(r01 >> 16);
        st[tr_slot[2]] = (short)(r23 & 0xffffu);
        st[tr_slot[3]] = (short)(r23 >> 16);
        __builtin_amdgcn_fence(__ATOMIC_RELEASE, "wavefront");
        __builtin_amdgcn_wave_barrier();
        __builtin_amdgcn_fence(__ATOMIC_ACQUIRE, "wavefront");
        ops = reinterpret_cast<const uint2 *>(st)[l];
        q16_pass(ops.x, ops.y, KC, odd, negm, o, ymax, ymin);
        __builtin_amdgcn_wave_barrier();
        constexpr unsigned CAP = 1u << 30;
        unsigned es = min((unsigned)energy, CAP), rs = min((unsigned)renergy, CAP);
#define HVC_Q16_STEP(CTRL)                                                                       \
        es = min(es + (unsigned)__builtin_amdgcn_mov_dpp((int)es, CTRL, 0xf, 0xf, true), CAP); \
        rs = min(rs + (unsigned)__builtin_amdgcn_mov_dpp((int)rs, CTRL, 0xf, 0xf, true), CAP);
        HVC_Q16_STEP(0xB1)
        HVC_Q16_STEP(0x4E)
        HVC_Q16_STEP(0x141)
        HVC_Q16_STEP(0x140)
#undef HVC_Q16_STEP
        const bool lbad = (es > (unsigned)P.ethr_packed[br.qtab]) | (rs >= (unsigned)GUARD_RE) | (ymax > GUARD_Y) |
                          (ymin < -GUARD_Y);
        const bool bad = ((__ballot(lbad) >> (lane & 48)) & 0xffffull) != 0;
        unsigned px01 = 0, px23 = 0;
        ashr14_sat_pack2<0>(px01, o[0], o[1]);
        ashr14_sat_pack2<0>(px23, o[2], o[3]);
        tile[oc[0]][bi][r] = (uint8_t)(px01 & 0xffu);
        tile[oc[1]][bi][r] = (uint8_t)((px01 >> 8) & 0xffu);
        tile[oc[2]][bi][r] = (uint8_t)(px23 & 0xffu);
        tile[oc[3]][bi][r] = (uint8_t)((px23 >> 8) & 0xffu);
        if (l == 0) badflag[bi] = (uint8_t)(bad && exists);
    }
    __syncthreads();
    const bool bad = badflag[lane] != 0;
    if (active && !bad) {
#pragma unroll
        for (int j = 0; j < 8; j++) {
            const uint2 px = *reinterpret_cast<const uint2 *>(&tile[j][lane][0]);
            store_row8(P.pixels + br.pix_idx + (size_t)j * br.stride, px.x, px.y);
        }
    }
    const bool flag = active && bad;
    const unsigned long long m = __ballot(flag);
    if (m) {
        const int wl = lane & 63;
        unsigned base = 0;
        if (wl == 0) base = atomicAdd(P.fix_count, (unsigned)__popcll(m));
        base = __shfl(base, 0);
        if (flag) {
            unsigned idx = base + (unsigned)__popcll(m & ((1ull << wl) - 1ull));
            P.fix_list[idx] = ((unsigned)blockIdx.y * (unsigned)P.tiles_per_frame + blockIdx.x) * HVC_TILE + lane;
        }
    }
}

template <bool WRAP63>
__device__ __forceinline__ void decode_block_wide(const unsigned (&w)[32], const int *__restrict__ q, bool has_dc, int64_t dc,
                                                  unsigned (&out)[8][2]) {
    int64_t v[64];
#pragma unroll
    for (int r = 0; r < 8; r++) {
        uint64_t in[8];
#pragma unroll
        for (int i = 0; i < 8; i++) {
            const int zz = ZF[8 * r + i];
            const int c = (zz & 1) ? (int)w[zz >> 1] >> 16 : (int)(short)(w[zz >> 1] & 0xffffu);
            in[i] = (uint64_t)((int64_t)c * (int64_t)q[zz]);
        }
        if (r == 0 && has_dc) in[0] = (uint64_t)mul63(dc, (int64_t)q[0]);
        int64_t o[8];
        idct8_wide<false, WRAP63>(in, o);
#pragma unroll
        for (int i = 0; i < 8; i++) v[8 * r + i] = o[i];
    }
#pragma unroll
    for (int j = 0; j < 8; j++) out[j][0] = out[j][1] = 0;
#pragma unroll
    for (int c = 0; c < 8; c++) {
        uint64_t in[8];
#pragma unroll
        for (int j = 0; j < 8; j++) in[j] = (uint64_t)v[8 * j + c];
        int64_t o[8];
        idct8_wide<true, WRAP63>(in, o);
#pragma unroll
        for (int j = 0; j < 8; j++) {
            const uint64_t y = (uint64_t)o[j] + 128u;
            const unsigned px = y <= 255u ? (unsigned)y : ((int64_t)y < 0 ? 0u : 255u);
            out[j][c >> 2] |= px << (8 * (c & 3));
        }
    }
}

__device__ __forceinline__ void load_block_dwords(const int16_t *cf, unsigned (&w)[32]) {
    const uint4 *src = reinterpret_cast<const uint4 *>(cf);
#pragma unroll
    for (int j = 0; j < 8; j++) {
        const uint4 t = src[j];
        w[4 * j + 0] = t.x;
        w[4 * j + 1] = t.y;
        w[4 * j + 2] = t.z;
        w[4 * j + 3] = t.w;
    }
}

#ifndef HVC_FIXUP_WGS
#define HVC_FIXUP_WGS 512
#endif
#ifndef HVC_FIXUP_LANES
#define HVC_FIXUP_LANES 256
#endif
__global__ __launch_bounds__(HVC_FIXUP_LANES) void k_decode_wide(DecodeParams P, const unsigned *count, const unsigned *list,
                                                                 const long long *dc_list) {
    const unsigned long long n = (unsigned long long)*count;
    if (blockIdx.x == 0 && threadIdx.x == 0) {
        if (P.fix_count_next) *P.fix_count_next = 0;
        if (P.wide_total) {
            if (P.wide_first == 2) atomicAdd(P.wide_total, n);
            else *P.wide_total = P.wide_first ? n : *P.wide_total + n;
        }
    }
    for (unsigned long long i = (unsigned long long)blockIdx.x * blockDim.x + threadIdx.x; i < n;
         i += (unsigned long long)gridDim.x * blockDim.x) {
        const unsigned long long id = list[i];
        const int lane = (int)(id % HVC_TILE);
        const unsigned long long t = id / HVC_TILE;
        const int tile = (int)(t % (unsigned)P.tiles_per_frame);
        const int frame = (int)(t / (unsigned)P.tiles_per_frame);
        if (frame >= P.n_frames) continue;
        BlockRef br;
        if (!locate(P, frame, tile, lane, br)) continue;
        unsigned w[32], out[8][2];
        load_block_dwords(P.coefs + br.coef_idx, w);
        int64_t dc = 0;
        if (P.dc_plane)
            dc = (int64_t)P.dc_plane[(size_t)frame * P.dc_fs + ((br.coef_idx - (size_t)frame * P.coef_fs) >> 6)];
        if (dc_list) dc = (int64_t)dc_list[i];
        decode_block_wide<true>(w, P.qt + br.qtab * 64, P.dc_plane != nullptr || dc_list != nullptr, dc, out);
#pragma unroll
        for (int j = 0; j < 8; j++) store_row8(P.pixels + br.pix_idx + (size_t)j * br.stride, out[j][0], out[j][1]);
    }
}

__global__ __launch_bounds__(HVC_TILE) void k_decode_wide_all(DecodeParams P) {
    BlockRef br;
    const int lane = threadIdx.x;
    unsigned wframe, wtile;
    xcd_work(P.xcd_map, P.xcd_magic, wframe, wtile);
    const bool active = locate(P, (int)wframe, (int)wtile, lane, br);
    unsigned w[32], out[8][2];
    load_block_dwords(P.coefs + br.coef_idx, w);
    int64_t dc = 0;
    if (P.dc_plane) dc = (int64_t)P.dc_plane[(size_t)wframe * P.dc_fs + ((br.coef_idx - (size_t)wframe * P.coef_fs) >> 6)];
    decode_block_wide<false>(w, P.qt + br.qtab * 64, P.dc_plane != nullptr, dc, out);
    if (active) {
#pragma unroll
        for (int j = 0; j < 8; j++) store_row8(P.pixels + br.pix_idx + (size_t)j * br.stride, out[j][0], out[j][1]);
    }
}

struct Ref444 {
    int p, bx, by;
    bool active;
    bool store;
};

__device__ __forceinline__ Ref444 locate444(const Decode444Params &P, int tile, int lane, int wgs, int tw) {
    Ref444 r;
    if (tile < P.y_tiles) {
        const Plane444K &K = P.pl[0];
        const int n = K.cbw * K.cbh;
        int b = tile * wgs + lane;
        r.active = b < n;
        b = r.active ? b : n - 1;
        const unsigned by = K.cbw == 1 ? (unsigned)b : __umulhi((unsigned)b, P.y_magic);
        r.p = 0;
        r.by = (int)by;
        r.bx = b - (int)by * K.cbw;
        r.store = r.active;
    } else {
        int t = tile - P.y_tiles;
        const int per = P.c_tiles_x * P.c_tiles_y;
        r.p = 1;
        if (t >= per) {
            r.p = 2;
            t -= per;
        }
        const unsigned ty = P.c_tiles_x == 1 ? (unsigned)t : __umulhi((unsigned)t, P.c_magic);
        const unsigned tx = (unsigned)t - ty * (unsigned)P.c_tiles_x;
        const Plane444K &K = P.pl[r.p];
        const int lx = lane & (tw - 1), ly = lane / tw;
        const int bx = (int)tx * (tw - 1) + lx, by = (int)ty * HVC_444_TILE_BH + ly;
        r.active = bx < K.cbw && by < K.cbh;
        r.store = r.active && (lx < tw - 1 || bx == K.cbw - 1);
        r.bx = min(bx, K.cbw - 1);
        r.by = min(by, K.cbh - 1);
    }
    return r;
}

template <bool ALIGNED>
__device__ __forceinline__ void store16(uint8_t *row, int x0, int w, unsigned d0, unsigned d1, unsigned d2,
                                        unsigned d3) {
    if (ALIGNED) {
        typedef unsigned u4s __attribute__((ext_vector_type(4)));
        const u4s t = {d0, d1, d2, d3};
        __builtin_nontemporal_store(t, reinterpret_cast<u4s *>(row + x0));
    } else {
        const unsigned d[4] = {d0, d1, d2, d3};
        for (int i = 0; i < 16; i++)
            if (x0 + i < w) row[x0 + i] = (uint8_t)(d[i >> 2] >> (8 * (i & 3)));
    }
}

struct RowQ {
    unsigned a0, a1, hc0, hc1, hf0, hf1, x0, x1;
};
template <int K>
__device__ __forceinline__ RowQ rowq(unsigned a0, unsigned a1, unsigned next, unsigned m0, unsigned m1) {
    RowQ q;
    q.a0 = a0;
    q.a1 = a1;
    unsigned b0 = __builtin_amdgcn_alignbyte(a1, a0, 1);
    unsigned b1 = __builtin_amdgcn_perm(next, a1, ((unsigned)(4 + K) << 24) | 0x030201u);
// ... 35 lines not shown
#define HVC_444_ATTR
#endif
template <bool ALIGNED, bool DCP, int NW>
__global__ __launch_bounds__(HVC_TILE * NW, 4 / NW) HVC_444_ATTR void k_decode_444(Decode444Params P) {
    constexpr int WGS = HVC_TILE * NW, TW = HVC_444_TILE_BW * NW;
    __shared__ uint4 edge[WGS];
    const int lane = threadIdx.x;
    unsigned wframe, wtile;
    xcd_work(P.xcd_map, P.xcd_magic, wframe, wtile);
    const int tile = (int)wtile + P.tile0;
    const bool chroma = tile >= P.y_tiles;
    if (P.skip && P.skip == (chroma ? 2 : 1)) return;
    const Ref444 r = locate444(P, tile, lane, WGS, TW);
    const Plane444K &K = P.pl[r.p];
    const size_t in_frame = K.coef_off + ((size_t)r.by * K.bw + r.bx) * 64;
    const uint4 *src = reinterpret_cast<const uint4 *>(P.coefs + (size_t)wframe * P.coef_fs + in_frame);
    const unsigned *__restrict__ qp = P.qpair + K.qtab * 32;
    PackedGuard g;
    unsigned out[8][2];
    int16_t dcv = 0;
    if (DCP) dcv = P.dc_plane[(size_t)wframe * P.dc_fs + (in_frame >> 6)];
#if HVC_TRAFFIC_ONLY == 2
    const int hvc_src_stride = 1;
#endif
    HVC_DECODE_BLOCK_PACKED(src, qp, out, g, if (DCP) w[0] = with_dc(w[0], dcv););
    const bool bad = packed_guard_failed(g, P.ethr_packed[K.qtab]);

    const size_t W = (size_t)P.width;
    uint8_t *plane = P.out + (size_t)wframe * P.out_fs + K.out_off;
    const int lasty = K.ah - 1 - r.by * 8;
    if (!chroma) {
        if (r.active && !bad) {
            uint8_t *p = plane + (size_t)r.by * 8 * W + (size_t)r.bx * 8;
#pragma unroll
            for (int j = 0; j < 8; j++) {
                if (j <= lasty) {
                    if (ALIGNED) {
                        store_row8(p + (size_t)j * W, out[j][0], out[j][1]);
                    } else {
                        for (int i = 0; i < 8; i++)
                            if (r.bx * 8 + i < K.aw) p[(size_t)j * W + i] = (uint8_t)(out[j][i >> 2] >> (8 * (i & 3)));
                    }
                }
            }
        }
    } else {
        constexpr unsigned B0 = 0x0c0c0400u, JOIN = 0x05040100u;
        const unsigned c0 = __builtin_amdgcn_perm(__builtin_amdgcn_perm(out[3][0], out[2][0], B0),
                                                  __builtin_amdgcn_perm(out[1][0], out[0][0], B0), JOIN);
        const unsigned c1 = __builtin_amdgcn_perm(__builtin_amdgcn_perm(out[7][0], out[6][0], B0),
                                                  __builtin_amdgcn_perm(out[5][0], out[4][0], B0), JOIN);
        edge[lane] = make_uint4(out[0][0], out[0][1], c0, c1);
        __syncthreads();
        const uint4 rt = edge[min(lane + 1, WGS - 1)];
        const uint4 dn = edge[min(lane + TW, WGS - 1)];
        const unsigned dg = edge[min(lane + TW + 1, WGS - 1)].x;
        const int lastx = K.aw - 1 - r.bx * 8;
        const unsigned long long mm = lastx >= 8 ? 0ull : (~0ull << (8 * max(lastx, 0)));
        const unsigned m0 = (unsigned)mm, m1 = (unsigned)(mm >> 32);
        if (r.store && !bad) {
            uint8_t *p = plane + (size_t)r.by * 16 * W;
            const int x0 = r.bx * 16;
            const RowQ q0 = rowq<0>(out[0][0], out[0][1], rt.z, m0, m1);
            const RowQ q1 = rowq<1>(out[1][0], out[1][1], rt.z, m0, m1);
            const RowQ q2 = rowq<2>(out[2][0], out[2][1], rt.z, m0, m1);
            const RowQ q3 = rowq<3>(out[3][0], out[3][1], rt.z, m0, m1);
            const RowQ q4 = rowq<0>(out[4][0], out[4][1], rt.w, m0, m1);
            const RowQ q5 = rowq<1>(out[5][0], out[5][1], rt.w, m0, m1);
            const RowQ q6 = rowq<2>(out[6][0], out[6][1], rt.w, m0, m1);
            const RowQ q7 = rowq<3>(out[7][0], out[7][1], rt.w, m0, m1);
            const RowQ q8 = rowq<0>(dn.x, dn.y, dg, m0, m1);
            if (0 <= lasty) emit_rows444<ALIGNED>(p + 0 * W, W, x0, q0, q1, lasty == 0);
            if (1 <= lasty) emit_rows444<ALIGNED>(p + 2 * W, W, x0, q1, q2, lasty == 1);
            if (2 <= lasty) emit_rows444<ALIGNED>(p + 4 * W, W, x0, q2, q3, lasty == 2);
            if (3 <= lasty) emit_rows444<ALIGNED>(p + 6 * W, W, x0, q3, q4, lasty == 3);
            if (4 <= lasty) emit_rows444<ALIGNED>(p + 8 * W, W, x0, q4, q5, lasty == 4);
            if (5 <= lasty) emit_rows444<ALIGNED>(p + 10 * W, W, x0, q5, q6, lasty == 5);
            if (6 <= lasty) emit_rows444<ALIGNED>(p + 12 * W, W, x0, q6, q7, lasty == 6);
            if (7 <= lasty) emit_rows444<ALIGNED>(p + 14 * W, W, x0, q7, q8, lasty == 7);
        }
    }
    const bool flag = r.store && bad;
    const unsigned long long m = __ballot(flag);
    if (m) {
        const int wl = lane & 63;
        unsigned base = 0;
        if (wl == 0) base = atomicAdd(P.fix_count, (unsigned)__popcll(m));
        base = __shfl(base, 0);
        if (flag) {
            unsigned idx = base + (unsigned)__popcll(m & ((1ull << wl) - 1ull));
            P.fix_list[idx] = (wframe * (unsigned)P.tiles_per_frame + (unsigned)tile) * WGS + lane;
        }
    }
}

__global__ __launch_bounds__(64) void k_decode_wide_444(Decode444Params P, const unsigned *count, const unsigned *list,
                                                        unsigned long long total, const long long *dc_list) {
    const unsigned long long n = list ? (unsigned long long)*count : total;
    if (blockIdx.x == 0 && threadIdx.x == 0) {
        if (P.fix_count_next) *P.fix_count_next = 0;
        if (P.wide_total && list) {
            if (P.wide_first == 2) atomicAdd(P.wide_total, n);
            else *P.wide_total = P.wide_first ? n : *P.wide_total + n;
        }
    }
    for (unsigned long long i = (unsigned long long)blockIdx.x * 64 + threadIdx.x; i < n;
         i += (unsigned long long)gridDim.x * 64) {
        const unsigned long long id = list ? list[i] : i;
        const unsigned wgs = (unsigned)(HVC_TILE * P.nw);
        const int lane = (int)(id % wgs);
        const unsigned long long t = id / wgs;
        const int tile = (int)(t % (unsigned)P.tiles_per_frame);
        const size_t frame = (size_t)(t / (unsigned)P.tiles_per_frame);
        if (frame >= (size_t)P.n_frames) continue;
        const Ref444 r = locate444(P, tile, lane, (int)wgs, HVC_444_TILE_BW * P.nw);
        if (!r.store) continue;
        const Plane444K &K = P.pl[r.p];
        const size_t in_frame = K.coef_off + ((size_t)r.by * K.bw + r.bx) * 64;
        unsigned w[32], out[8][2];
        load_block_dwords(P.coefs + frame * P.coef_fs + in_frame, w);
        int64_t dc = 0;
        if (P.dc_plane) dc = (int64_t)P.dc_plane[frame * P.dc_fs + (in_frame >> 6)];
        if (dc_list) dc = (int64_t)dc_list[i];
        decode_block_wide<true>(w, P.qt + K.qtab * 64, P.dc_plane != nullptr || dc_list != nullptr, dc, out);
        uint8_t *plane = P.out + frame * P.out_fs + K.out_off;
        const int step = r.p == 0 ? 1 : 2;
#pragma unroll
        for (int j = 0; j < 8; j++)
#pragma unroll
            for (int i2 = 0; i2 < 8; i2++) {
                const int x = r.bx * 8 + i2, y = r.by * 8 + j;
                if (x >= K.aw || y >= K.ah) continue;
                plane[(size_t)(y * step) * (size_t)P.width + (size_t)(x * step)] = (uint8_t)(out[j][i2 >> 2] >> (8 * (i2 & 3)));
            }
    }
}

__device__ __forceinline__ unsigned avg2u(unsigned a, unsigned b) { return (a + b + 1) >> 1; }
__device__ __forceinline__ unsigned avg4u(unsigned a, unsigned b, unsigned c, unsigned d) { return (a + b + c + d + 2) >> 2; }

__device__ __forceinline__ void reinterp_sample(uint8_t *plane, size_t W, int aw, int ah, int c, int r) {
    const int c2 = min(c + 1, aw - 1), r2 = min(r + 1, ah - 1);
    const unsigned a = plane[(size_t)(2 * r) * W + 2 * c], b = plane[(size_t)(2 * r) * W + 2 * c2];
    const unsigned cc = plane[(size_t)(2 * r2) * W + 2 * c], d = plane[(size_t)(2 * r2) * W + 2 * c2];
    plane[(size_t)(2 * r) * W + 2 * c + 1] = (uint8_t)avg2u(a, b);
    plane[(size_t)(2 * r + 1) * W + 2 * c] = (uint8_t)avg2u(a, cc);
    plane[(size_t)(2 * r + 1) * W + 2 * c + 1] = (uint8_t)avg4u(a, b, cc, d);
}

__device__ __forceinline__ void reinterp_hseam16(uint8_t *plane, size_t W, int aw, int r, int t) {
    const uint8_t *re = plane + (size_t)(2 * r) * W + 16 * (size_t)t;
    const uint8_t *rn = re + 2 * W;
    const uint4 A = *reinterpret_cast<const uint4 *>(re), C = *reinterpret_cast<const uint4 *>(rn);
    const bool more = 8 * t + 8 < aw;
    const unsigned a[4] = {A.x, A.y, A.z, A.w}, c[4] = {C.x, C.y, C.z, C.w};
    const unsigned an = more ? re[16] : (A.w >> 16) & 0xffu, cn = more ? rn[16] : (C.w >> 16) & 0xffu;
    unsigned o[4];
#pragma unroll
    for (int k = 0; k < 4; k++) {
        const unsigned a0 = a[k] & 0xffu, a1 = (a[k] >> 16) & 0xffu, c0 = c[k] & 0xffu, c1 = (c[k] >> 16) & 0xffu;
        const unsigned a2 = k < 3 ? a[k + 1] & 0xffu : an, c2 = k < 3 ? c[k + 1] & 0xffu : cn;
        o[k] = avg2u(a0, c0) | (avg4u(a0, a1, c0, c1) << 8) | (avg2u(a1, c1) << 16) | (avg4u(a1, a2, c1, c2) << 24);
    }
    *reinterpret_cast<uint4 *>(plane + (size_t)(2 * r + 1) * W + 16 * (size_t)t) = make_uint4(o[0], o[1], o[2], o[3]);
}

template <bool VEC>
__global__ __launch_bounds__(256) void k_reinterp_444(Decode444Params P, const unsigned *count, const unsigned *list,
                                                      int all) {
    const Plane444K &K1 = P.pl[1];
    const int aw = K1.aw, ah = K1.ah;
    const size_t W = (size_t)P.width;
    const size_t frame = blockIdx.y;
    const long long tid = (long long)blockIdx.x * 256 + threadIdx.x;
    if (all) {
        const long long per = (long long)aw * ah;
        if (tid < 2 * per) {
            const int p = tid >= per ? 2 : 1;
            const long long s = tid - (p - 1) * per;
            reinterp_sample(P.out + frame * P.out_fs + P.pl[p].out_off, W, aw, ah, (int)(s % aw), (int)(s / aw));
        }
        return;
    }
    const int nhs = P.c_tiles_y - 1;
    const int hw = VEC ? aw / 8 : aw;
    const long long per = (long long)nhs * hw;
    if (tid < 2 * per) {
        const int p = tid >= per ? 2 : 1;
        const long long s = tid - (p - 1) * per;
        uint8_t *plane = P.out + frame * P.out_fs + P.pl[p].out_off;
        const int r = (int)(s / hw) * (8 * HVC_444_TILE_BH) + 8 * HVC_444_TILE_BH - 1;
        if (r + 1 < ah) {
            if (VEC)
                reinterp_hseam16(plane, W, aw, r, (int)(s % hw));
            else
                reinterp_sample(plane, W, aw, ah, (int)(s % hw), r);
        }
    }
    const unsigned long long n = (unsigned long long)*count * 81ull;
    const unsigned long long nthreads = (unsigned long long)gridDim.x * gridDim.y * 256ull;
    for (unsigned long long i = (unsigned long long)blockIdx.y * gridDim.x * 256ull + (unsigned long long)tid; i < n;
         i += nthreads) {
        const unsigned long long id = list[i / 81];
        const int k = (int)(i % 81);
        const unsigned wgs = (unsigned)(HVC_TILE * P.nw);
        const int lane = (int)(id % wgs);
        const unsigned long long t = id / wgs;
        const int tile = (int)(t % (unsigned)P.tiles_per_frame);
        const size_t f = (size_t)(t / (unsigned)P.tiles_per_frame);
        if (f >= (size_t)P.n_frames) continue;
        const Ref444 rr = locate444(P, tile, lane, (int)wgs, HVC_444_TILE_BW * P.nw);
        if (!rr.store || rr.p == 0) continue;
        const int c = rr.bx * 8 - 1 + k % 9, r = rr.by * 8 - 1 + k / 9;
        if (c < 0 || r < 0 || c >= aw || r >= ah) continue;
        reinterp_sample(P.out + f * P.out_fs + P.pl[rr.p].out_off, W, aw, ah, c, r);
    }
}


__device__ __forceinline__ int vmul24(int k, int x) {
    int d;
    asm("v_mul_i32_i24 %0, %1, %2" : "=v"(d) : "s"(k), "v"(x));
    return d;
}
__device__ __forceinline__ int vmad24(int k, int x, int acc) {
    int d;
    asm("v_mad_i32_i24 %0, %1, %2, %3" : "=v"(d) : "s"(k), "v"(x), "v"(acc));
    return d;
}
#ifndef HVC_ENCODE_MULHI
#define HVC_ENCODE_MULHI 1
#endif
#ifndef HVC_ENCODE_QMAGIC
#define HVC_ENCODE_QMAGIC 1
#endif
__device__ __forceinline__ int vmulhi24(int k, int x) {
    int d;
    asm("v_mul_hi_i32_i24 %0, %1, %2" : "=v"(d) : "s"(k), "v"(x));
    return d;
}
__device__ __forceinline__ int c4(int f, int g) { return vmul24(362, f + g) >> 9; }
__device__ __forceinline__ int c4m(int f, int g) { return vmul24(362, f - g) >> 9; }
__device__ __forceinline__ int c62(int f, int g) { return vmad24(473, g, vmul24(196, f)) >> 9; }
__device__ __forceinline__ int c71(int f, int g) { return vmad24(502, g, vmul24(100, f)) >> 9; }
__device__ __forceinline__ int c35(int f, int g) { return vmad24(284, g, vmul24(426, f)) >> 9; }
__device__ __forceinline__ int c62n(int f, int g) { return vmad24(-473, g, vmul24(196, f)) >> 9; }
__device__ __forceinline__ int c71n(int f, int g) { return vmad24(-502, g, vmul24(100, f)) >> 9; }
__device__ __forceinline__ int c35n(int f, int g) { return vmad24(-284, g, vmul24(426, f)) >> 9; }

template <bool LS>
__device__ __forceinline__ void fdct_tail(int a0, int a1, int a2, int a3, int c0, int c1, int c2, int c3, int &p0,
                                          int &p1, int &p2, int &p3, int &p4, int &p5, int &p6, int &p7) {
#if HVC_ENCODE_MULHI
    constexpr int C4S = 362 << 14;
    const int b0s = (a0 + a3) << 9, b1s = (a1 + a2) << 9, b2 = a1 - a2, b3 = a0 - a3;
    p0 = vmulhi24(C4S, LS ? b0s + b1s - (1024 << 9) : b0s + b1s);
    p4 = vmulhi24(C4S, b0s - b1s);
    p2 = c62(b2, b3);
    p6 = c62n(b3, b2);
    const int c2s = c2 << 9;
    int b0 = vmulhi24(C4S, vmad24(-512, c1, c2s));
    int b1 = vmulhi24(C4S, vmad24(512, c1, c2s));
#else
    int b0 = LS ? a0 + a3 - 512 : a0 + a3, b1 = LS ? a1 + a2 - 512 : a1 + a2, b2 = a1 - a2, b3 = a0 - a3;
    p0 = c4(b0, b1);
    p4 = c4m(b0, b1);
    p2 = c62(b2, b3);
    p6 = c62n(b3, b2);
    b0 = c4m(c2, c1);
    b1 = c4(c2, c1);
#endif
    a0 = c0 + b0;
    a1 = c0 - b0;
    a2 = c3 - b1;
    a3 = c3 + b1;
    p1 = c71(a0, a3);
    p5 = c35(a1, a2);
    p3 = c35n(a2, a1);
    p7 = c71n(a3, a0);
}

template <int BYTE>
__device__ __forceinline__ int add_bytes(unsigned a, unsigned b) {
    int d;
    if (BYTE == 0) asm("v_add_u32_sdwa %0, %1, %2 dst_sel:DWORD dst_unused:UNUSED_PAD src0_sel:BYTE_0 src1_sel:BYTE_0" : "=v"(d) : "v"(a), "v"(b));
    if (BYTE == 1) asm("v_add_u32_sdwa %0, %1, %2 dst_sel:DWORD dst_unused:UNUSED_PAD src0_sel:BYTE_1 src1_sel:BYTE_1" : "=v"(d) : "v"(a), "v"(b));
    if (BYTE == 2) asm("v_add_u32_sdwa %0, %1, %2 dst_sel:DWORD dst_unused:UNUSED_PAD src0_sel:BYTE_2 src1_sel:BYTE_2" : "=v"(d) : "v"(a), "v"(b));
    if (BYTE == 3) asm("v_add_u32_sdwa %0, %1, %2 dst_sel:DWORD dst_unused:UNUSED_PAD src0_sel:BYTE_3 src1_sel:BYTE_3" : "=v"(d) : "v"(a), "v"(b));
    return d;
}
template <int BYTE>
__device__ __forceinline__ int sub_bytes(unsigned a, unsigned b) {
    int d;
    if (BYTE == 0) asm("v_sub_u32_sdwa %0, %1, %2 dst_sel:DWORD dst_unused:UNUSED_PAD src0_sel:BYTE_0 src1_sel:BYTE_0" : "=v"(d) : "v"(a), "v"(b));
    if (BYTE == 1) asm("v_sub_u32_sdwa %0, %1, %2 dst_sel:DWORD dst_unused:UNUSED_PAD src0_sel:BYTE_1 src1_sel:BYTE_1" : "=v"(d) : "v"(a), "v"(b));
    if (BYTE == 2) asm("v_sub_u32_sdwa %0, %1, %2 dst_sel:DWORD dst_unused:UNUSED_PAD src0_sel:BYTE_2 src1_sel:BYTE_2" : "=v"(d) : "v"(a), "v"(b));
    if (BYTE == 3) asm("v_sub_u32_sdwa %0, %1, %2 dst_sel:DWORD dst_unused:UNUSED_PAD src0_sel:BYTE_3 src1_sel:BYTE_3" : "=v"(d) : "v"(a), "v"(b));
    return d;
}
// ... 207 lines not shown
    const unsigned an = last ? 0u : s1[8], bn = last ? 0u : s2[8];
    const unsigned m1 = last ? 0xff000000u : 0u;
    const RowQ cur = rowq<0>(a.x, a.y, an, 0u, m1), nxt = rowq<0>(b.x, b.y, bn, 0u, m1);
    emit_rows444<true>(dst + (size_t)(2 * row) * P.dst_stride, P.dst_stride, 16 * g, cur, nxt, false);
}

__device__ __forceinline__ unsigned absdiff_u8x4(unsigned a, unsigned b) {
    unsigned r = 0;
#pragma unroll
    for (int k = 0; k < 4; k++) {
        const int d = (int)((a >> (8 * k)) & 0xffu) - (int)((b >> (8 * k)) & 0xffu);
        r |= (unsigned)(d < 0 ? -d : d) << (8 * k);
    }
    return r;
}
__global__ __launch_bounds__(HVC_TILE) void k_abs_error(EncodeParams P, const uint8_t *recon, uint8_t *error) {
    BlockRef br;
    if (!locate(P, blockIdx.y, blockIdx.x, threadIdx.x, br)) return;
#pragma unroll
    for (int j = 0; j < 8; j++) {
        const size_t at = br.pix_idx + (size_t)j * br.stride;
        const uint2 a = *reinterpret_cast<const uint2 *>(P.pixels + at), b = *reinterpret_cast<const uint2 *>(recon + at);
        *reinterpret_cast<uint2 *>(error + at) = make_uint2(absdiff_u8x4(b.x, a.x), absdiff_u8x4(b.y, a.y));
    }
}
hipError_t launch_abs_error(const EncodeParams &P, const uint8_t *recon, uint8_t *error, hipStream_t s) {
    if (P.n_frames <= 0 || P.tiles_per_frame <= 0) return hipSuccess;
    hipLaunchKernelGGL(k_abs_error, dim3((unsigned)P.tiles_per_frame, (unsigned)P.n_frames, 1), dim3(HVC_TILE), 0, s, P, recon, error);
    return hipGetLastError();
}

__global__ __launch_bounds__(256) void k_checksum(const uint8_t *data, size_t record_bytes, size_t record_stride,
                                                  unsigned long long *sums) {
    const uint8_t *rec = data + (size_t)blockIdx.y * record_stride;
    const size_t vec = ((uintptr_t)rec & 15) == 0 ? record_bytes / 16 : 0;
    unsigned long long acc = 0;
    for (size_t v = (size_t)blockIdx.x * 256 + threadIdx.x; v < vec; v += (size_t)gridDim.x * 256) {
        const uint4 q = reinterpret_cast<const uint4 *>(rec)[v];
        const unsigned w[4] = {q.x, q.y, q.z, q.w};
        unsigned s0 = 0, s1 = 0;
#pragma unroll
        for (int k = 0; k < 16; k++) {
            const unsigned b = ((w[k >> 2] >> (8 * (k & 3))) & 0xffu) + 1u;
            s0 += b;
            s1 += (unsigned)k * b;
        }
        acc += (2ull * (16ull * v) + 1ull) * s0 + 2ull * s1;
    }
    if (blockIdx.x == 0)
        for (size_t i = vec * 16 + threadIdx.x; i < record_bytes; i += 256) acc += (2ull * i + 1ull) * ((unsigned long long)rec[i] + 1ull);
    acc *= HVC_CHECKSUM_MUL;
#pragma unroll
    for (int o = 32; o > 0; o >>= 1) acc += __shfl_xor(acc, o);
    if ((threadIdx.x & 63) == 0 && acc) atomicAdd(&sums[blockIdx.y], acc);
}

hipError_t launch_checksum(const uint8_t *data, size_t record_bytes, size_t record_stride, int n_records,
                           unsigned long long *sums, hipStream_t s) {
    if (n_records <= 0) return hipSuccess;
    hipError_t e = hipMemsetAsync(sums, 0, (size_t)n_records * sizeof(unsigned long long), s);
    if (e != hipSuccess) return e;
    if (record_bytes == 0) return hipSuccess;
    const size_t pieces = (record_bytes / 16 + 255) / 256;
    size_t gx = pieces < 1 ? 1 : pieces;
    const size_t want = (size_t)(4096 + n_records - 1) / (size_t)n_records;
    if (gx > want) gx = want;
    hipLaunchKernelGGL(k_checksum, dim3((unsigned)gx, (unsigned)n_records, 1), dim3(256), 0, s, data, record_bytes,
                       record_stride, sums);
    return hipGetLastError();
}


hipError_t launch_decode(const DecodeParams &P, hipStream_t s, hipEvent_t k0, hipEvent_t k1) {
    if (P.n_frames <= 0 || P.tiles_per_frame <= 0) return hipSuccess;
    hipError_t e;
    dim3 grid((unsigned)P.tiles_per_frame, (unsigned)P.n_frames, 1);
    if (k0 && (e = hipEventRecord(k0, s)) != hipSuccess) return e;
    static const int env_sel = [] {
        const char *v = getenv("HVC_DECODE_KERNEL");
        return !v ? 0 : (v[0] == 'v' && v[1] == '2') ? 1 : (v[0] == 'q') ? 3 : 0;
    }();
    const int sel = P.kernel_sel ? P.kernel_sel : P.dc_plane ? 0 : env_sel;
    if (P.dc_plane && sel != 0) return hipErrorInvalidValue;
    if (sel == 3)
        hipLaunchKernelGGL(k_decode_q16, grid, dim3(HVC_TILE), 0, s, P);
    else if (sel == 1)
        hipLaunchKernelGGL(k_decode_fast, grid, dim3(HVC_TILE), 0, s, P);
    else {
        static const unsigned pad = [] { const char *v = getenv("HVC_DEC_LDS_PAD"); return v ? (unsigned)atoi(v) : 0u; }();
        DecodeParams Q = P;
        Q.xcd_map = xcd_map_for(grid.x, grid.y, Q.xcd_magic);
        if (P.dc_plane)
            hipLaunchKernelGGL(k_decode_packed<true>, grid, dim3(HVC_TILE), pad, s, Q);
        else
            hipLaunchKernelGGL(k_decode_packed<false>, grid, dim3(HVC_TILE), pad, s, Q);
    }
    e = hipGetLastError();
    if (e != hipSuccess) return e;
    if (k1 && (e = hipEventRecord(k1, s)) != hipSuccess) return e;
    hipLaunchKernelGGL(k_decode_wide, dim3(HVC_FIXUP_WGS), dim3(HVC_FIXUP_LANES), 0, s, P, P.fix_count, P.fix_list, (const long long *)nullptr);
    return hipGetLastError();
}

hipError_t launch_decode_dcfix(const DecodeParams &P, const unsigned *count, const unsigned *ids, const long long *dcs,
                               hipStream_t s) {
    DecodeParams Q = P;
    Q.fix_count_next = nullptr;
    Q.wide_total = nullptr;
    hipLaunchKernelGGL(k_decode_wide, dim3(64), dim3(64), 0, s, Q, count, ids, dcs);
    return hipGetLastError();
}

hipError_t launch_decode_444_dcfix(const Decode444Params &P, const unsigned *count, const unsigned *ids, const long long *dcs,
                                   unsigned n_host, hipStream_t s) {
    Decode444Params Q = P;
    Q.fix_count_next = nullptr;
    Q.wide_total = nullptr;
    hipLaunchKernelGGL(k_decode_wide_444, dim3(64), dim3(64), 0, s, Q, count, ids, 0ull, dcs);
    const size_t W = (size_t)P.width;
    const bool aligned = (W % 16 == 0) && (P.out_fs % 16 == 0) && ((uintptr_t)P.out % 16 == 0);
    const long long hw = aligned ? P.pl[1].aw / 8 : P.pl[1].aw;
    const long long seams = 2 * (long long)(P.c_tiles_y - 1) * hw;
    const long long want = seams > (long long)n_host * 81 ? seams : (long long)n_host * 81;
    const dim3 rgrid((unsigned)((want + 255) / 256) ? (unsigned)((want + 255) / 256) : 1u, (unsigned)P.n_frames, 1);
    if (aligned)
        hipLaunchKernelGGL(k_reinterp_444<true>, rgrid, dim3(256), 0, s, Q, count, ids, 0);
    else
        hipLaunchKernelGGL(k_reinterp_444<false>, rgrid, dim3(256), 0, s, Q, count, ids, 0);
    return hipGetLastError();
}

hipError_t launch_decode_wide_only(const DecodeParams &P, hipStream_t s, hipEvent_t k0, hipEvent_t k1) {
    if (P.n_frames <= 0 || P.tiles_per_frame <= 0) return hipSuccess;
    hipError_t e;
    const dim3 grid((unsigned)P.tiles_per_frame, (unsigned)P.n_frames, 1);
    DecodeParams Q = P;
    Q.xcd_map = xcd_map_for(grid.x, grid.y, Q.xcd_magic);
    if (k0 && (e = hipEventRecord(k0, s)) != hipSuccess) return e;
    hipLaunchKernelGGL(k_decode_wide_all, grid, dim3(HVC_TILE), 0, s, Q);
    if ((e = hipGetLastError()) != hipSuccess) return e;
    if (k1 && (e = hipEventRecord(k1, s)) != hipSuccess) return e;
    return hipSuccess;
}

void plan_decode_444(Decode444Params &P, bool aligned) {
    const int cbw = P.pl[1].cbw;
    P.nw = !aligned || cbw <= HVC_444_TILE_BW ? 1 : cbw <= 2 * HVC_444_TILE_BW ? 2 : 4;
    const int wgs = HVC_TILE * P.nw, tw = HVC_444_TILE_BW * P.nw;
    P.y_tiles = (P.pl[0].cbw * P.pl[0].cbh + wgs - 1) / wgs;
    P.y_magic = (unsigned)(((1ull << 32) + P.pl[0].cbw - 1) / P.pl[0].cbw);
    P.c_tiles_x = cbw <= tw ? 1 : (cbw - 1 + (tw - 1) - 1) / (tw - 1);
    P.c_tiles_y = (P.pl[1].cbh + HVC_444_TILE_BH - 1) / HVC_444_TILE_BH;
    P.c_magic = (unsigned)(((1ull << 32) + P.c_tiles_x - 1) / P.c_tiles_x);
    P.tiles_per_frame = P.y_tiles + 2 * P.c_tiles_x * P.c_tiles_y;
}

template <bool ALIGNED, int NW>
static void launch_444_kernel(const Decode444Params &Q, dim3 grid, unsigned pad, hipStream_t s) {
    if (Q.dc_plane)
        hipLaunchKernelGGL((k_decode_444<ALIGNED, true, NW>), grid, dim3(HVC_TILE * NW), pad, s, Q);
    else
        hipLaunchKernelGGL((k_decode_444<ALIGNED, false, NW>), grid, dim3(HVC_TILE * NW), pad, s, Q);
}

hipError_t launch_decode_444(const Decode444Params &P, bool wide_only, hipStream_t s, hipEvent_t k0, hipEvent_t k1) {
    if (P.n_frames <= 0 || P.tiles_per_frame <= 0) return hipSuccess;
    if (P.nw != 1 && P.nw != 2 && P.nw != 4) return hipErrorInvalidValue;
    const dim3 grid((unsigned)P.tiles_per_frame, (unsigned)P.n_frames, 1);
    const long long per_plane = (long long)P.pl[1].aw * P.pl[1].ah;
    if (wide_only) {
        const unsigned long long total = (unsigned long long)P.n_frames * P.tiles_per_frame * HVC_TILE * P.nw;
        if (k0) (void)hipEventRecord(k0, s);
        hipLaunchKernelGGL(k_decode_wide_444, dim3(4096), dim3(64), 0, s, P, (const unsigned *)nullptr,
                           (const unsigned *)nullptr, total, (const long long *)nullptr);
        if (k1) (void)hipEventRecord(k1, s);
        hipLaunchKernelGGL(k_reinterp_444<false>, dim3((unsigned)((2 * per_plane + 255) / 256), (unsigned)P.n_frames, 1),
                           dim3(256), 0, s, P, (const unsigned *)P.fix_count, (const unsigned *)P.fix_list, 1);
        return hipGetLastError();
    }
    const size_t W = (size_t)P.width;
    const bool aligned = (W % 16 == 0) && (P.out_fs % 16 == 0) && ((uintptr_t)P.out % 16 == 0);
    if (k0) (void)hipEventRecord(k0, s);
    static const int only = [] { const char *v = getenv("HVC_444_ONLY"); return !v ? 0 : v[0] == 'l' ? 2 : v[0] == 'c' ? 1 : 0; }();
    Decode444Params Q = P;
    Q.skip = only;
    Q.xcd_map = xcd_map_for((unsigned)(P.tiles_per_frame - P.tile0), (unsigned)P.n_frames, Q.xcd_magic, true);
    static const unsigned pad = [] { const char *v = getenv("HVC_444_LDS_PAD"); return v ? (unsigned)atoi(v) : 0u; }();
    if (!aligned && P.nw != 1) return hipErrorInvalidValue;
    const dim3 cgrid((unsigned)(P.tiles_per_frame - P.tile0), (unsigned)P.n_frames, 1);
    if (!aligned)
        launch_444_kernel<false, 1>(Q, cgrid, 0, s);
    else if (P.nw == 1)
        launch_444_kernel<true, 1>(Q, cgrid, pad, s);
    else if (P.nw == 2)
        launch_444_kernel<true, 2>(Q, cgrid, pad, s);
    else
        launch_444_kernel<true, 4>(Q, cgrid, pad, s);
    if (k1) (void)hipEventRecord(k1, s);
    hipLaunchKernelGGL(k_decode_wide_444, dim3(256), dim3(64), 0, s, P, (const unsigned *)P.fix_count,
                       (const unsigned *)P.fix_list, 0ull, (const long long *)nullptr);
    const long long hw = aligned ? P.pl[1].aw / 8 : P.pl[1].aw;
    const long long seams = 2 * (long long)(P.c_tiles_y - 1) * hw;
    const dim3 rgrid((unsigned)((seams + 255) / 256) ? (unsigned)((seams + 255) / 256) : 1u, (unsigned)P.n_frames, 1);
    if (aligned)
        hipLaunchKernelGGL(k_reinterp_444<true>, rgrid, dim3(256), 0, s, P, (const unsigned *)P.fix_count,
                           (const unsigned *)P.fix_list, 0);
    else
        hipLaunchKernelGGL(k_reinterp_444<false>, rgrid, dim3(256), 0, s, P, (const unsigned *)P.fix_count,
                           (const unsigned *)P.fix_list, 0);
    return hipGetLastError();
}

hipError_t launch_encode(const EncodeParams &P, hipStream_t s, hipEvent_t k0, hipEvent_t k1) {
    if (P.n_frames <= 0 || P.tiles_per_frame <= 0) return hipSuccess;
    hipError_t e;
    dim3 grid((unsigned)P.tiles_per_frame, (unsigned)P.n_frames, 1);
    if (k0 && (e = hipEventRecord(k0, s)) != hipSuccess) return e;
    static const unsigned pad = [] { const char *v = getenv("HVC_ENC_LDS_PAD"); return v ? (unsigned)atoi(v) : 0u; }();
    EncodeParams Q = P;
    Q.xcd_map = xcd_map_for(grid.x, grid.y, Q.xcd_magic);
    hipLaunchKernelGGL(k_encode, grid, dim3(HVC_TILE), pad, s, Q);
    e = hipGetLastError();
    if (e != hipSuccess) return e;
    if (k1 && (e = hipEventRecord(k1, s)) != hipSuccess) return e;
    return hipSuccess;
}

hipError_t launch_upsample420(const UpsampleParams &P, hipStream_t s) {
    if (P.n_planes <= 0 || P.cw <= 0 || P.ch <= 0) return hipSuccess;
    long long total = (long long)((P.cw + 3) >> 2) * P.ch;
    dim3 grid((unsigned)((total + 255) / 256), (unsigned)P.n_planes, 1);
    const bool vec = (P.cw % 4 == 0) && (P.src_stride % 4 == 0) && (P.dst_stride % 8 == 0) && (P.src_ps % 4 == 0) &&
                     (P.dst_ps % 8 == 0) && ((uintptr_t)P.src % 4 == 0) && ((uintptr_t)P.dst % 8 == 0);
    const bool x8 = (P.cw % 8 == 0) && (P.src_stride % 8 == 0) && (P.dst_stride % 16 == 0) && (P.src_ps % 8 == 0) &&
                    (P.dst_ps % 16 == 0) && ((uintptr_t)P.src % 8 == 0) && ((uintptr_t)P.dst % 16 == 0);
    if (x8) {
        const long long n8 = (long long)(P.cw >> 3) * P.ch;
        UpsampleParams Q = P;
        Q.xcd_map = xcd_map_for((unsigned)((n8 + 255) / 256), (unsigned)P.n_planes, Q.xcd_magic);
        hipLaunchKernelGGL(k_upsample420_x8, dim3((unsigned)((n8 + 255) / 256), (unsigned)P.n_planes, 1), dim3(256), 0,
                           s, Q);
    } else if (vec)
        hipLaunchKernelGGL(k_upsample420<true>, grid, dim3(256), 0, s, P);
    else
        hipLaunchKernelGGL(k_upsample420<false>, grid, dim3(256), 0, s, P);
    return hipGetLastError();
}

}
```

### video-coding_amd/csrc/hvc_mixed.h

```cpp
#ifndef HVC_MIXED_H
#define HVC_MIXED_H

#include <hip/hip_runtime.h>

#include "hvc_mixed_plan.h"

namespace hvc {

struct MixedParams {
    const int16_t *coefs;
    uint8_t *pixels;
    const MixedPlaneK *planes;
    const MixedTableK *tables;
    const unsigned *map;
    unsigned n_units;
    int all_wide;
    unsigned *fix_count, *fix_count_next, *fix_list;
    unsigned long long *wide_total;
    int wide_first;
    int xcd_map;
    unsigned xcd_magic;
};

hipError_t launch_decode_mixed(const MixedParams &P, hipStream_t s, hipEvent_t k0 = nullptr, hipEvent_t k1 = nullptr);

}
#endif
```

### video-coding_amd/csrc/hvc_mixed.hip

```cpp
#include <hip/hip_runtime.h>
#include <stdint.h>

#include "hvc_idct_spec.h"
#include "hvc_kernels.h"
#include "hvc_mixed.h"

namespace hvc {
namespace {

#define HVC_MIXED_LANES (HVC_MIXED_UNIT * HVC_MIXED_GROUP)

__device__ constexpr int MZF[64] = {0,  1,  5,  6,  14, 15, 27, 28, 2,  4,  7,  13, 16, 26, 29, 42, 3,  8,  12, 17, 25, 30,
                                    41, 43, 9,  11, 18, 24, 31, 40, 44, 53, 10, 19, 23, 32, 39, 45, 52, 54, 20, 22, 33, 38,
                                    46, 51, 55, 60, 21, 34, 37, 47, 50, 56, 59, 61, 35, 36, 48, 49, 57, 58, 62, 63};

typedef short m_short2 __attribute__((ext_vector_type(2)));
typedef unsigned short m_ushort2 __attribute__((ext_vector_type(2)));
typedef unsigned m_uint2 __attribute__((ext_vector_type(2)));

template <int ADD>
__device__ __forceinline__ int m_dot2(unsigned pair, unsigned k) {
    static_assert(ADD == 0 || ADD == 4, "inline constants only");
    int d;
    if (ADD == 0)
// ... 83 lines not shown
    do {                                                                                                   \
        _Pragma("unroll") for (int d = 0; d < 32; d++) (G).energy = m_dot2_sat((W)[d], (W)[d], (G).energy); \
        unsigned cA[8], cB[8], cC[8], cZ[8];                                                               \
        {                                                                                                  \
            int ra[8], rb[8];                                                                              \
            m_row<HVC_PAIR_A_LO>((W), (QP) + 4 * HVC_PAIR_A_LO, ra, (G));                                  \
            m_row<HVC_PAIR_A_HI>((W), (QP) + 4 * HVC_PAIR_A_HI, rb, (G));                                  \
            _Pragma("unroll") for (int c = 0; c < 8; c++) cA[c] = m_pack_rows(ra[c], rb[c], (G));          \
            m_row<HVC_PAIR_B_LO>((W), (QP) + 4 * HVC_PAIR_B_LO, ra, (G));                                  \
            m_row<HVC_PAIR_B_HI>((W), (QP) + 4 * HVC_PAIR_B_HI, rb, (G));                                  \
            _Pragma("unroll") for (int c = 0; c < 8; c++) cB[c] = m_pack_rows(ra[c], rb[c], (G));          \
            m_row<HVC_PAIR_C_LO>((W), (QP) + 4 * HVC_PAIR_C_LO, ra, (G));                                  \
            m_row<HVC_PAIR_C_HI>((W), (QP) + 4 * HVC_PAIR_C_HI, rb, (G));                                  \
            _Pragma("unroll") for (int c = 0; c < 8; c++) cC[c] = m_pack_rows(ra[c], rb[c], (G));          \
            m_row<HVC_PAIR_Z_LO>((W), (QP) + 4 * HVC_PAIR_Z_LO, ra, (G));                                  \
            m_row<HVC_PAIR_Z_HI>((W), (QP) + 4 * HVC_PAIR_Z_HI, rb, (G));                                  \
            _Pragma("unroll") for (int c = 0; c < 8; c++) cZ[c] = m_pack_rows(ra[c], rb[c], (G));          \
        }                                                                                                  \
        _Pragma("unroll") for (int c = 0; c < 8; c += 2) {                                                 \
            int ca[8], cb[8];                                                                              \
            m_col(cA[c], cB[c], cC[c], cZ[c], ca, (G));                                                    \
            m_col(cA[c + 1], cB[c + 1], cC[c + 1], cZ[c + 1], cb, (G));                                    \
            _Pragma("unroll") for (int j = 0; j < 8; j++) {                                                \
                if ((c & 2) == 0)                                                                          \
                    m_pack2<0>((OUT)[j][c >> 2], ca[j], cb[j]);                                            \
                else                                                                                       \
                    m_pack2<1>((OUT)[j][c >> 2], ca[j], cb[j]);                                            \
            }                                                                                              \
        }                                                                                                  \
    } while (0)

struct MixedRef {
    const int16_t *coef;
    uint8_t *pix;
    size_t stride;
};
__device__ __forceinline__ MixedRef mixed_block(const MixedParams &P, const MixedPlaneK &K, int b) {
    const unsigned by = K.bw == 1 ? (unsigned)b : __umulhi((unsigned)b, K.magic);
    const unsigned bx = (unsigned)b - by * (unsigned)K.bw;
    MixedRef r;
    r.stride = (size_t)K.stride;
    r.coef = P.coefs + (size_t)K.coef_base + (size_t)b * 64;
    r.pix = P.pixels + (size_t)K.pix_base + (size_t)by * 8 * r.stride + (size_t)bx * 8;
    return r;
}

__global__ __launch_bounds__(HVC_MIXED_LANES, 4) void k_decode_mixed(MixedParams P) {
    unsigned wf, wt;
    xcd_work(P.xcd_map, P.xcd_magic, wf, wt);
    const unsigned group = wf * gridDim.x + wt;
    const int lane = threadIdx.x & (HVC_MIXED_UNIT - 1);
    const unsigned unit = (unsigned)__builtin_amdgcn_readfirstlane((int)(group * HVC_MIXED_GROUP + (threadIdx.x >> 6)));
    if (unit >= P.n_units) return;
    const MixedPlaneK &K = P.planes[P.map[unit]];
    const MixedTableK &T = P.tables[K.table];
    int b = (int)(unit - K.unit0) * HVC_MIXED_UNIT + lane;
    const bool active = b < K.nblk;
    b = active ? b : K.nblk - 1;
    const MixedRef br = mixed_block(P, K, b);
    bool flag = active;
    if (!(P.all_wide | T.wide)) {
        const uint4 *src = reinterpret_cast<const uint4 *>(br.coef);
        unsigned w[32];
#pragma unroll
        for (int j = 0; j < 8; j++) {
            const uint4 t = src[j];
            w[4 * j + 0] = t.x;
            w[4 * j + 1] = t.y;
            w[4 * j + 2] = t.z;
            w[4 * j + 3] = t.w;
        }
        MGuard g;
        unsigned out[8][2];
        const unsigned *__restrict__ qp = T.qpair;
        HVC_MX_DECODE_BLOCK(w, qp, out, g);
        const bool bad = g.failed(T.ethr_packed);
        if (active && !bad) {
#pragma unroll
            for (int j = 0; j < 8; j++) m_store_row(br.pix + (size_t)j * br.stride, out[j][0], out[j][1]);
        }
        flag = active && bad;
    }
    const unsigned long long m = __ballot(flag);
    if (m) {
        unsigned base = 0;
        if (lane == 0) base = atomicAdd(P.fix_count, (unsigned)__popcll(m));
        base = __shfl(base, 0);
        if (flag) P.fix_list[base + (unsigned)__popcll(m & ((1ull << lane) - 1ull))] = unit * HVC_MIXED_UNIT + (unsigned)lane;
    }
}

template <bool COL>
__device__ __forceinline__ void m_idct8_wide(const uint64_t (&b)[8], int64_t (&o)[8]) {
    typedef uint64_t u64;
    constexpr u64 w1 = HVC_W1, w2 = HVC_W2, w3 = HVC_W3, w5 = HVC_W5, w6 = HVC_W6, w7 = HVC_W7;
    constexpr u64 R = COL ? 4 : 0;
    constexpr int RS = COL ? 3 : 0, S = COL ? 14 : 8;
    auto asr = [](u64 x, int s) { return (u64)((int64_t)x >> s); };
    u64 x0 = COL ? b[0] * 256u + 8192u : b[0] * 2048u + 128u;
    u64 x1 = COL ? b[4] * 256u : b[4] * 2048u;
    u64 x2 = b[6], x3 = b[2], x4 = b[1], x5 = b[7], x6 = b[5], x7 = b[3];
    u64 x8 = w7 * (x4 + x5) + R;
    x4 = asr(x8 + (w1 - w7) * x4, RS);
    x5 = asr(x8 - (w1 + w7) * x5, RS);
    x8 = w3 * (x6 + x7) + R;
    x6 = asr(x8 - (w3 - w5) * x6, RS);
    x7 = asr(x8 - (w3 + w5) * x7, RS);
    x8 = x0 + x1;
    x0 = x0 - x1;
    x1 = w6 * (x3 + x2) + R;
    x2 = asr(x1 - (w2 + w6) * x2, RS);
    x3 = asr(x1 + (w2 - w6) * x3, RS);
    x1 = x4 + x6;
    x4 = x4 - x6;
    x6 = x5 + x7;
    x5 = x5 - x7;
    x7 = x8 + x3;
    x8 = x8 - x3;
    x3 = x0 + x2;
    x0 = x0 - x2;
    x2 = asr(181u * (x4 + x5) + 128u, 8);
    x4 = asr(181u * (x4 - x5) + 128u, 8);
    o[0] = (int64_t)asr(x7 + x1, S);
    o[1] = (int64_t)asr(x3 + x2, S);
    o[2] = (int64_t)asr(x0 + x4, S);
    o[3] = (int64_t)asr(x8 + x6, S);
    o[4] = (int64_t)asr(x8 - x6, S);
    o[5] = (int64_t)asr(x0 - x4, S);
    o[6] = (int64_t)asr(x3 - x2, S);
    o[7] = (int64_t)asr(x7 - x1, S);
}

__device__ __forceinline__ void m_block_wide(const unsigned (&w)[32], const int *__restrict__ q, unsigned (&out)[8][2]) {
    int64_t v[64];
#pragma unroll
    for (int r = 0; r < 8; r++) {
        uint64_t in[8];
#pragma unroll
        for (int i = 0; i < 8; i++) {
            const int zz = MZF[8 * r + i];
            const int c = (zz & 1) ? (int)w[zz >> 1] >> 16 : (int)(short)(w[zz >> 1] & 0xffffu);
            in[i] = (uint64_t)((int64_t)c * (int64_t)q[zz]);
        }
        int64_t o[8];
        m_idct8_wide<false>(in, o);
#pragma unroll
        for (int i = 0; i < 8; i++) v[8 * r + i] = o[i];
    }
#pragma unroll
    for (int j = 0; j < 8; j++) out[j][0] = out[j][1] = 0;
#pragma unroll
    for (int c = 0; c < 8; c++) {
        uint64_t in[8];
#pragma unroll
        for (int j = 0; j < 8; j++) in[j] = (uint64_t)v[8 * j + c];
        int64_t o[8];
        m_idct8_wide<true>(in, o);
#pragma unroll
        for (int j = 0; j < 8; j++) {
            const uint64_t y = (uint64_t)o[j] + 128u;
            const unsigned px = y <= 255u ? (unsigned)y : ((int64_t)y < 0 ? 0u : 255u);
            out[j][c >> 2] |= px << (8 * (c & 3));
        }
    }
}

#define HVC_MIXED_WIDE_WGS 512
#define HVC_MIXED_WIDE_LANES 256
__global__ __launch_bounds__(HVC_MIXED_WIDE_LANES) void k_decode_mixed_wide(MixedParams P) {
    const unsigned long long n = (unsigned long long)*P.fix_count;
    if (blockIdx.x == 0 && threadIdx.x == 0) {
        if (P.fix_count_next) *P.fix_count_next = 0;
        if (P.wide_total) *P.wide_total = P.wide_first ? n : *P.wide_total + n;
    }
    for (unsigned long long i = (unsigned long long)blockIdx.x * blockDim.x + threadIdx.x; i < n;
         i += (unsigned long long)gridDim.x * blockDim.x) {
        const unsigned id = P.fix_list[i];
        const unsigned unit = id / HVC_MIXED_UNIT, lane = id % HVC_MIXED_UNIT;
        if (unit >= P.n_units) continue;
        const MixedPlaneK K = P.planes[P.map[unit]];
        if (unit < K.unit0) continue;
        const unsigned long long b = (unsigned long long)(unit - K.unit0) * HVC_MIXED_UNIT + lane;
        if (b >= (unsigned long long)K.nblk) continue;
        const MixedRef br = mixed_block(P, K, (int)b);
        const uint4 *src = reinterpret_cast<const uint4 *>(br.coef);
        unsigned w[32], out[8][2];
#pragma unroll
        for (int j = 0; j < 8; j++) {
            const uint4 t = src[j];
            w[4 * j + 0] = t.x;
            w[4 * j + 1] = t.y;
            w[4 * j + 2] = t.z;
            w[4 * j + 3] = t.w;
        }
        m_block_wide(w, P.tables[K.table].qt, out);
#pragma unroll
        for (int j = 0; j < 8; j++) m_store_row(br.pix + (size_t)j * br.stride, out[j][0], out[j][1]);
    }
}

}

hipError_t launch_decode_mixed(const MixedParams &P, hipStream_t s, hipEvent_t k0, hipEvent_t k1) {
    if (P.n_units == 0) return hipSuccess;
    hipError_t e;
    const unsigned groups = (P.n_units + HVC_MIXED_GROUP - 1) / HVC_MIXED_GROUP;
    MixedParams Q = P;
    Q.xcd_map = xcd_map_for(groups, 1, Q.xcd_magic);
    if (k0 && (e = hipEventRecord(k0, s)) != hipSuccess) return e;
    hipLaunchKernelGGL(k_decode_mixed, dim3(groups), dim3(HVC_MIXED_LANES), 0, s, Q);
    if ((e = hipGetLastError()) != hipSuccess) return e;
    if (k1 && (e = hipEventRecord(k1, s)) != hipSuccess) return e;
    hipLaunchKernelGGL(k_decode_mixed_wide, dim3(HVC_MIXED_WIDE_WGS), dim3(HVC_MIXED_WIDE_LANES), 0, s, Q);
    return hipGetLastError();
}

}
```

Before: 1.349 million.

## Shard fix-list atomic counters across 64 cache-line-separated segments

Replaces the single global atomic counter used to append wide-fallback block ids with 64 sharded counters, each padded to its own line, selected by workgroup index. Consumers walk the per-shard segments, and the first workgroup sums and clears the shard counters. The aim is to cut atomic contention on one address across XCDs in the decode kernels. In exchange the fix-list allocation is larger, segments are padded, and the fixup kernels do a little more bookkeeping.

```diff
diff --git a/video-coding_amd/csrc/hvc_capi.hip b/video-coding_amd/csrc/hvc_capi.hip
--- a/video-coding_amd/csrc/hvc_capi.hip
+++ b/video-coding_amd/csrc/hvc_capi.hip
@@ -541,7 +541,7 @@
     if (!c || !count) return HVC_E_INVALID_ARG;
     DeviceGuard g(c->device);
     unsigned long long v = 0;
-    HIPCHK(c, hipMemcpyAsync(&v, c->d_fix_count + 2, sizeof v, hipMemcpyDeviceToHost, c->stream));
+    HIPCHK(c, hipMemcpyAsync(&v, fix_wide_total(c), sizeof v, hipMemcpyDeviceToHost, c->stream));
     HIPCHK(c, hipStreamSynchronize(c->stream));
     *count = c->wide_host >= 0 ? (uint64_t)c->wide_host : (uint64_t)v;
     return HVC_OK;
@@ -832,11 +832,12 @@
     const int per = frames_per_launch_capped(n_frames, L.blocks_per_frame, ids_per_frame);
     const bool has_wide = o.wide && !o.wide->empty();
     if (has_wide && (unsigned long long)n_frames * ids_per_frame >= (1ull << 32)) return HVC_E_TOO_LARGE;
+    if (ids_per_frame >= (1ull << 32)) return HVC_E_TOO_LARGE;
     DeviceGuard g(c->device);
     if (!g.ok) return fail_hip(c, hipErrorInvalidDevice);
 
     const bool twin = o.arith == HVC_ARITH_HARDCAML;
-    if ((r = reserve_fix_list(c, twin ? 0 : (size_t)((unsigned long long)per * ids_per_frame)))) return r;
+    if ((r = reserve_fix_list(c, twin ? 0 : hvc::fix_list_entries((unsigned long long)per * (unsigned long long)L.tiles_per_frame, HVC_TILE)))) return r;
 
     hvc::DecodeParams P;
     fill_geometry(P, L, coef_fs, pixel_fs, n_frames);
@@ -939,7 +940,7 @@
     hvc::DecodeParams P;
     fill_geometry(P, L, coef_fs, pixel_fs, n_frames);
     for (int i = 0; i < n_qtabs * 64; i++) P.qt[i] = (int)qtabs[i];
-    P.wide_total = reinterpret_cast<unsigned long long *>(c->d_fix_count + 2);
+    P.wide_total = fix_wide_total(c);
     wide_total_begin(c);
     bool rows_on_dwords = ((n_frames > 1 ? pixel_fs : 0) & 3) == 0;
     for (int i = 0; i < n_comp; i++) rows_on_dwords &= ((comps[i].plane_offset | comps[i].stride) & 3) == 0;
@@ -1174,7 +1175,7 @@
     const int per = frames_per_launch_capped(n_frames, L.blocks_per_frame, ids_per_frame);
     const bool has_wide = o.wide && !o.wide->empty();
     if (has_wide && (unsigned long long)n_frames * ids_per_frame >= (1ull << 32)) return HVC_E_TOO_LARGE;
-    const unsigned long long ids = (unsigned long long)per * ids_per_frame;
+    if (ids_per_frame >= (1ull << 32)) return HVC_E_TOO_LARGE;
     DeviceGuard g(c->device);
     if (!g.ok) return fail_hip(c, hipErrorInvalidDevice);
     int ethr_unused[HVC_MAX_QTABS];
@@ -1182,8 +1183,9 @@
     bool wide_only = c->decode_kernel == 2;
     for (int i = 0; i < n_qtabs * 64; i++) wide_only |= qtabs[i] > 255;
     const int split = (aligned && !wide_only && c->decode_kernel == 0 && height % 8 == 0 && P.pl[0].cbw == P.pl[0].bw) ? fused444_mode() : 0;
-    const size_t luma_ids = split ? (size_t)per * (size_t)((P.pl[0].cbw * P.pl[0].cbh + HVC_TILE - 1) / HVC_TILE) * HVC_TILE : 0;
-    if ((r = reserve_fix_list(c, luma_ids + (size_t)ids))) return r;
+    const size_t list_444 = hvc::fix_list_entries((unsigned long long)per * (unsigned long long)P.tiles_per_frame, (unsigned)(HVC_TILE * P.nw));
+    const size_t list_luma = split ? hvc::fix_list_entries((unsigned long long)per * (unsigned long long)((P.pl[0].cbw * P.pl[0].cbh + HVC_TILE - 1) / HVC_TILE), HVC_TILE) : 0;
+    if ((r = reserve_fix_list(c, list_444 + list_luma))) return r;
     P.fix_list = c->d_fix_list;
     wide_total_begin(c);
     if (split == 2 && !c->side_stream) {
@@ -1216,10 +1218,10 @@
         prepare_tables(qtabs, n_qtabs, Y.qt, Y.ethr, Y.ethr_packed, Y.qpair);
         Y.dc_plane = Q.dc_plane;
         Y.dc_fs = Q.dc_fs;
-        Y.fix_count = c->d_fix_count + 4 + c->fix_phase_l;
-        Y.fix_count_next = c->d_fix_count + 4 + (c->fix_phase_l ^ 1);
-        Y.fix_list = c->d_fix_list + (size_t)ids;
-        Y.wide_total = reinterpret_cast<unsigned long long *>(c->d_fix_count + 2);
+        Y.fix_count = fix_counter_set(c, 2 + c->fix_phase_l);
+        Y.fix_count_next = fix_counter_set(c, 2 + (c->fix_phase_l ^ 1));
+        Y.fix_list = c->d_fix_list + list_444;
+        Y.wide_total = fix_wide_total(c);
         fix_assign(c, Q);
         Q.tile0 = Q.y_tiles;
         hipStream_t ys = c->stream;
diff --git a/video-coding_amd/csrc/hvc_capi_mixed.hip b/video-coding_amd/csrc/hvc_capi_mixed.hip
--- a/video-coding_amd/csrc/hvc_capi_mixed.hip
+++ b/video-coding_amd/csrc/hvc_capi_mixed.hip
@@ -69,7 +69,8 @@
     int r;
     if (plan.map.empty()) return HVC_OK;
     if (((uintptr_t)d_coefs & 15) || ((uintptr_t)d_pixels & 7)) return HVC_E_ALIGNMENT;
-    if ((r = reserve_mixed_fix_list(c, plan.map.size() * HVC_MIXED_UNIT))) return r;
+    if ((unsigned long long)plan.map.size() * HVC_MIXED_UNIT > (1ull << 32)) return HVC_E_TOO_LARGE;
+    if ((r = reserve_mixed_fix_list(c, hvc::mixed_fix_list_entries(plan.map.size())))) return r;
     hvc::MixedParams P;
     std::memset(&P, 0, sizeof P);
     if ((r = upload_plan(c, plan, P))) return r;
diff --git a/video-coding_amd/csrc/hvc_ctx.h b/video-coding_amd/csrc/hvc_ctx.h
--- a/video-coding_amd/csrc/hvc_ctx.h
+++ b/video-coding_amd/csrc/hvc_ctx.h
@@ -28,7 +28,8 @@
 #include "hvc_scaled_spec.h"
 
 #define HVC_PROF_RING 64
-#define HVC_FIX_WORDS 8
+#define HVC_FIX_SET_WORDS (hvc::FIX_SHARDS * hvc::FIX_LINE)
+#define HVC_FIX_WORDS (hvc::FIX_LINE + 4 * HVC_FIX_SET_WORDS)
 
 struct hvc_ctx {
     int device = -1;
@@ -153,12 +154,14 @@
 
 int grow(hvc_ctx *c, void **p, size_t *cap, size_t need);
 
+inline unsigned *fix_counter_set(const hvc_ctx *c, int set) { return c->d_fix_count + hvc::FIX_LINE + (size_t)set * HVC_FIX_SET_WORDS; }
+inline unsigned long long *fix_wide_total(const hvc_ctx *c) { return reinterpret_cast<unsigned long long *>(c->d_fix_count); }
 template <class Params>
 inline void fix_assign(const hvc_ctx *c, Params &P) {
-    P.fix_count = c->d_fix_count + c->fix_phase;
-    P.fix_count_next = c->d_fix_count + (c->fix_phase ^ 1);
+    P.fix_count = fix_counter_set(c, c->fix_phase);
+    P.fix_count_next = fix_counter_set(c, c->fix_phase ^ 1);
     P.fix_list = c->d_fix_list;
-    P.wide_total = reinterpret_cast<unsigned long long *>(c->d_fix_count + 2);
+    P.wide_total = fix_wide_total(c);
     P.wide_first = c->wide_total_started ? 0 : 1;
 }
 inline void fix_commit(hvc_ctx *c) {
diff --git a/video-coding_amd/csrc/hvc_kernels.h b/video-coding_amd/csrc/hvc_kernels.h
--- a/video-coding_amd/csrc/hvc_kernels.h
+++ b/video-coding_amd/csrc/hvc_kernels.h
@@ -14,6 +14,19 @@
 #include "hvc_idct_spec.h"
 
 namespace hvc {
+
+#ifndef HVC_FIX_SHARDS
+#define HVC_FIX_SHARDS 64
+#endif
+constexpr unsigned FIX_SHARDS = HVC_FIX_SHARDS;
+constexpr unsigned FIX_LINE = 32;
+static_assert(FIX_SHARDS >= 8 && (FIX_SHARDS & (FIX_SHARDS - 1)) == 0, "a power of two, a multiple of the 8 XCDs");
+inline unsigned fix_seg_cap(unsigned long long workgroups, unsigned lanes, unsigned shards = FIX_SHARDS) {
+    return (unsigned)((workgroups + shards - 1) / shards * lanes);
+}
+inline size_t fix_list_entries(unsigned long long workgroups, unsigned lanes, unsigned shards = FIX_SHARDS) {
+    return (size_t)shards * fix_seg_cap(workgroups, lanes, shards);
+}
 
 static const unsigned char HVC_ZF[64] = {
     0,  1,  5,  6,  14, 15, 27, 28, 2,  4,  7,  13, 16, 26, 29, 42, 3,  8,  12, 17, 25, 30,
@@ -52,6 +65,7 @@
     int wide_first;
     int xcd_map;
     unsigned xcd_magic;
+    unsigned fix_shards, fix_seg_cap;
 };
 
 struct EncodeParams {
@@ -109,6 +123,7 @@
     int wide_first;
     int xcd_map;
     unsigned xcd_magic;
+    unsigned fix_shards, fix_seg_cap;
 };
 
 inline int xcd_map_run(bool fused = false) {
@@ -131,6 +146,38 @@
             tile = lin - frame * per;
         }
     }
+}
+__device__ __forceinline__ void fix_append(unsigned *count, unsigned *list, unsigned shards, unsigned seg_cap,
+                                           unsigned long long m, bool flag, int wl, unsigned id) {
+    const unsigned shard = (blockIdx.y * gridDim.x + blockIdx.x) & (shards - 1u);
+    unsigned base = 0;
+    if (wl == 0) base = atomicAdd(count + shard * FIX_LINE, (unsigned)__popcll(m));
+    base = __shfl(base, 0);
+    if (flag) list[(size_t)shard * seg_cap + base + (unsigned)__popcll(m & ((1ull << wl) - 1ull))] = id;
+}
+template <class F>
+__device__ __forceinline__ void fix_walk(const unsigned *count, const unsigned *list, unsigned shards, unsigned seg_cap,
+                                         unsigned w, unsigned n_wg, unsigned per, F f) {
+    const unsigned first = w & (shards - 1u);
+    const unsigned long long lanes = blockDim.x, rank = w / shards, share = (n_wg - first + shards - 1) / shards;
+    for (unsigned s = first; s < shards; s += n_wg) {
+        const unsigned long long n = (unsigned long long)count[s * FIX_LINE] * per;
+        const unsigned *seg = list + (size_t)s * seg_cap;
+        for (unsigned long long i = rank * lanes + threadIdx.x; i < n; i += share * lanes) f(i, seg[i / per]);
+    }
+}
+__device__ __forceinline__ unsigned long long fix_total_and_clear(const unsigned *count, unsigned *next, unsigned shards) {
+    __shared__ unsigned long long fix_sum;
+    if (threadIdx.x == 0) fix_sum = 0;
+    __syncthreads();
+    unsigned long long part = 0;
+    for (unsigned s = threadIdx.x; s < shards; s += blockDim.x) {
+        part += count[s * FIX_LINE];
+        if (next) next[s * FIX_LINE] = 0;
+    }
+    if (part) atomicAdd(&fix_sum, part);
+    __syncthreads();
+    return threadIdx.x == 0 ? fix_sum : 0ull;
 }
 #endif
 inline int xcd_map_for(unsigned per, unsigned n, unsigned &magic, bool fused = false) {
diff --git a/video-coding_amd/csrc/hvc_kernels.hip b/video-coding_amd/csrc/hvc_kernels.hip
--- a/video-coding_amd/csrc/hvc_kernels.hip
+++ b/video-coding_amd/csrc/hvc_kernels.hip
@@ -253,16 +253,9 @@
     }
     const bool flag = active && bad;
     const unsigned long long m = __ballot(flag);
-    if (m) {
-        const int wl = lane & 63;
-        unsigned base = 0;
-        if (wl == 0) base = atomicAdd(P.fix_count, (unsigned)__popcll(m));
-        base = __shfl(base, 0);
-        if (flag) {
-            unsigned idx = base + (unsigned)__popcll(m & ((1ull << wl) - 1ull));
-            P.fix_list[idx] = ((unsigned)blockIdx.y * (unsigned)P.tiles_per_frame + blockIdx.x) * HVC_TILE + lane;
-        }
-    }
+    if (m)
+        fix_append(P.fix_count, P.fix_list, P.fix_shards, P.fix_seg_cap, m, flag, lane & 63,
+                   ((unsigned)blockIdx.y * (unsigned)P.tiles_per_frame + blockIdx.x) * HVC_TILE + lane);
 }
 
 typedef short short2v __attribute__((ext_vector_type(2)));
@@ -461,16 +454,9 @@
     }
     const bool flag = active && bad;
     const unsigned long long m = __ballot(flag);
-    if (m) {
-        const int wl = lane & 63;
-        unsigned base = 0;
-        if (wl == 0) base = atomicAdd(P.fix_count, (unsigned)__popcll(m));
-        base = __shfl(base, 0);
-        if (flag) {
-            unsigned idx = base + (unsigned)__popcll(m & ((1ull << wl) - 1ull));
-            P.fix_list[idx] = (wframe * (unsigned)P.tiles_per_frame + wtile) * HVC_TILE + lane;
-        }
-    }
+    if (m)
+        fix_append(P.fix_count, P.fix_list, P.fix_shards, P.fix_seg_cap, m, flag, lane & 63,
+                   (wframe * (unsigned)P.tiles_per_frame + wtile) * HVC_TILE + lane);
 }
 
 constexpr int Q16_ITERS = HVC_TILE / 16;
@@ -620,16 +606,9 @@
     }
     const bool flag = active && bad;
     const unsigned long long m = __ballot(flag);
-    if (m) {
-        const int wl = lane & 63;
-        unsigned base = 0;
-        if (wl == 0) base = atomicAdd(P.fix_count, (unsigned)__popcll(m));
-        base = __shfl(base, 0);
-        if (flag) {
-            unsigned idx = base + (unsigned)__popcll(m & ((1ull << wl) - 1ull));
-            P.fix_list[idx] = ((unsigned)blockIdx.y * (unsigned)P.tiles_per_frame + blockIdx.x) * HVC_TILE + lane;
-        }
-    }
+    if (m)
+        fix_append(P.fix_count, P.fix_list, P.fix_shards, P.fix_seg_cap, m, flag, lane & 63,
+                   ((unsigned)blockIdx.y * (unsigned)P.tiles_per_frame + blockIdx.x) * HVC_TILE + lane);
 }
 
 template <bool WRAP63>
@@ -688,25 +667,22 @@
 #define HVC_FIXUP_LANES 256
 #endif
 __global__ __launch_bounds__(HVC_FIXUP_LANES) void k_decode_wide(DecodeParams P, const unsigned *count, const unsigned *list,
-                                                                 const long long *dc_list) {
-    const unsigned long long n = (unsigned long long)*count;
-    if (blockIdx.x == 0 && threadIdx.x == 0) {
-        if (P.fix_count_next) *P.fix_count_next = 0;
-        if (P.wide_total) {
+                                                                 unsigned shards, unsigned seg_cap, const long long *dc_list) {
+    if (blockIdx.x == 0 && (P.fix_count_next || P.wide_total)) {
+        const unsigned long long n = fix_total_and_clear(count, P.fix_count_next, shards);
+        if (threadIdx.x == 0 && P.wide_total) {
             if (P.wide_first == 2) atomicAdd(P.wide_total, n);
             else *P.wide_total = P.wide_first ? n : *P.wide_total + n;
         }
     }
-    for (unsigned long long i = (unsigned long long)blockIdx.x * blockDim.x + threadIdx.x; i < n;
-         i += (unsigned long long)gridDim.x * blockDim.x) {
-        const unsigned long long id = list[i];
+    fix_walk(count, list, shards, seg_cap, blockIdx.x, gridDim.x, 1u, [&](unsigned long long i, unsigned long long id) {
         const int lane = (int)(id % HVC_TILE);
         const unsigned long long t = id / HVC_TILE;
         const int tile = (int)(t % (unsigned)P.tiles_per_frame);
         const int frame = (int)(t / (unsigned)P.tiles_per_frame);
-        if (frame >= P.n_frames) continue;
+        if (frame >= P.n_frames) return;
         BlockRef br;
-        if (!locate(P, frame, tile, lane, br)) continue;
+        if (!locate(P, frame, tile, lane, br)) return;
         unsigned w[32], out[8][2];
         load_block_dwords(P.coefs + br.coef_idx, w);
         int64_t dc = 0;
@@ -716,7 +692,7 @@
         decode_block_wide<true>(w, P.qt + br.qtab * 64, P.dc_plane != nullptr || dc_list != nullptr, dc, out);
 #pragma unroll
         for (int j = 0; j < 8; j++) store_row8(P.pixels + br.pix_idx + (size_t)j * br.stride, out[j][0], out[j][1]);
-    }
+    });
 }
 
 __global__ __launch_bounds__(HVC_TILE) void k_decode_wide_all(DecodeParams P) {
@@ -918,58 +894,58 @@
     }
     const bool flag = r.store && bad;
     const unsigned long long m = __ballot(flag);
-    if (m) {
-        const int wl = lane & 63;
-        unsigned base = 0;
-        if (wl == 0) base = atomicAdd(P.fix_count, (unsigned)__popcll(m));
-        base = __shfl(base, 0);
-        if (flag) {
-            unsigned idx = base + (unsigned)__popcll(m & ((1ull << wl) - 1ull));
-            P.fix_list[idx] = (wframe * (unsigned)P.tiles_per_frame + (unsigned)tile) * WGS + lane;
-        }
-    }
+    if (m)
+        fix_append(P.fix_count, P.fix_list, P.fix_shards, P.fix_seg_cap, m, flag, lane & 63,
+                   (wframe * (unsigned)P.tiles_per_frame + (unsigned)tile) * WGS + lane);
+}
+
+__device__ __forceinline__ void decode_wide_444_block(const Decode444Params &P, unsigned long long id, bool has_dc_list, int64_t dcl) {
+    const unsigned wgs = (unsigned)(HVC_TILE * P.nw);
+    const int lane = (int)(id % wgs);
+    const unsigned long long t = id / wgs;
+    const int tile = (int)(t % (unsigned)P.tiles_per_frame);
+    const size_t frame = (size_t)(t / (unsigned)P.tiles_per_frame);
+    if (frame >= (size_t)P.n_frames) return;
+    const Ref444 r = locate444(P, tile, lane, (int)wgs, HVC_444_TILE_BW * P.nw);
+    if (!r.store) return;
+    const Plane444K &K = P.pl[r.p];
+    const size_t in_frame = K.coef_off + ((size_t)r.by * K.bw + r.bx) * 64;
+    unsigned w[32], out[8][2];
+    load_block_dwords(P.coefs + frame * P.coef_fs + in_frame, w);
+    int64_t dc = 0;
+    if (P.dc_plane) dc = (int64_t)P.dc_plane[frame * P.dc_fs + (in_frame >> 6)];
+    if (has_dc_list) dc = dcl;
+    decode_block_wide<true>(w, P.qt + K.qtab * 64, P.dc_plane != nullptr || has_dc_list, dc, out);
+    uint8_t *plane = P.out + frame * P.out_fs + K.out_off;
+    const int step = r.p == 0 ? 1 : 2;
+#pragma unroll
+    for (int j = 0; j < 8; j++)
+#pragma unroll
+        for (int i2 = 0; i2 < 8; i2++) {
+            const int x = r.bx * 8 + i2, y = r.by * 8 + j;
+            if (x >= K.aw || y >= K.ah) continue;
+            plane[(size_t)(y * step) * (size_t)P.width + (size_t)(x * step)] = (uint8_t)(out[j][i2 >> 2] >> (8 * (i2 & 3)));
+        }
 }
 
 __global__ __launch_bounds__(64) void k_decode_wide_444(Decode444Params P, const unsigned *count, const unsigned *list,
-                                                        unsigned long long total, const long long *dc_list) {
-    const unsigned long long n = list ? (unsigned long long)*count : total;
-    if (blockIdx.x == 0 && threadIdx.x == 0) {
-        if (P.fix_count_next) *P.fix_count_next = 0;
-        if (P.wide_total && list) {
+                                                        unsigned shards, unsigned seg_cap, unsigned long long total,
+                                                        const long long *dc_list) {
+    if (!list) {
+        for (unsigned long long i = (unsigned long long)blockIdx.x * 64 + threadIdx.x; i < total; i += (unsigned long long)gridDim.x * 64)
+            decode_wide_444_block(P, i, false, 0);
+        return;
+    }
+    if (blockIdx.x == 0 && (P.fix_count_next || P.wide_total)) {
+        const unsigned long long n = fix_total_and_clear(count, P.fix_count_next, shards);
+        if (threadIdx.x == 0 && P.wide_total) {
             if (P.wide_first == 2) atomicAdd(P.wide_total, n);
             else *P.wide_total = P.wide_first ? n : *P.wide_total + n;
         }
     }
-    for (unsigned long long i = (unsigned long long)blockIdx.x * 64 + threadIdx.x; i < n;
-         i += (unsigned long long)gridDim.x * 64) {
-        const unsigned long long id = list ? list[i] : i;
-        const unsigned wgs = (unsigned)(HVC_TILE * P.nw);
-        const int lane = (int)(id % wgs);
-        const unsigned long long t = id / wgs;
-        const int tile = (int)(t % (unsigned)P.tiles_per_frame);
-        const size_t frame = (size_t)(t / (unsigned)P.tiles_per_frame);
-        if (frame >= (size_t)P.n_frames) continue;
-        const Ref444 r = locate444(P, tile, lane, (int)wgs, HVC_444_TILE_BW * P.nw);
-        if (!r.store) continue;
-        const Plane444K &K = P.pl[r.p];
-        const size_t in_frame = K.coef_off + ((size_t)r.by * K.bw + r.bx) * 64;
-        unsigned w[32], out[8][2];
-        load_block_dwords(P.coefs + frame * P.coef_fs + in_frame, w);
-        int64_t dc = 0;
-        if (P.dc_plane) dc = (int64_t)P.dc_plane[frame * P.dc_fs + (in_frame >> 6)];
-        if (dc_list) dc = (int64_t)dc_list[i];
-        decode_block_wide<true>(w, P.qt + K.qtab * 64, P.dc_plane != nullptr || dc_list != nullptr, dc, out);
-        uint8_t *plane = P.out + frame * P.out_fs + K.out_off;
-        const int step = r.p == 0 ? 1 : 2;
-#pragma unroll
-        for (int j = 0; j < 8; j++)
-#pragma unroll
-            for (int i2 = 0; i2 < 8; i2++) {
-                const int x = r.bx * 8 + i2, y = r.by * 8 + j;
-                if (x >= K.aw || y >= K.ah) continue;
-                plane[(size_t)(y * step) * (size_t)P.width + (size_t)(x * step)] = (uint8_t)(out[j][i2 >> 2] >> (8 * (i2 & 3)));
-            }
-    }
+    fix_walk(count, list, shards, seg_cap, blockIdx.x, gridDim.x, 1u, [&](unsigned long long i, unsigned long long id) {
+        decode_wide_444_block(P, id, dc_list != nullptr, dc_list ? (int64_t)dc_list[i] : 0);
+    });
 }
 
 __device__ __forceinline__ unsigned avg2u(unsigned a, unsigned b) { return (a + b + 1) >> 1; }
@@ -1003,7 +979,7 @@
 
 template <bool VEC>
 __global__ __launch_bounds__(256) void k_reinterp_444(Decode444Params P, const unsigned *count, const unsigned *list,
-                                                      int all) {
+                                                      unsigned shards, unsigned seg_cap, int all) {
     const Plane444K &K1 = P.pl[1];
     const int aw = K1.aw, ah = K1.ah;
     const size_t W = (size_t)P.width;
@@ -1033,24 +1009,21 @@
                 reinterp_sample(plane, W, aw, ah, (int)(s % hw), r);
         }
     }
-    const unsigned long long n = (unsigned long long)*count * 81ull;
-    const unsigned long long nthreads = (unsigned long long)gridDim.x * gridDim.y * 256ull;
-    for (unsigned long long i = (unsigned long long)blockIdx.y * gridDim.x * 256ull + (unsigned long long)tid; i < n;
-         i += nthreads) {
-        const unsigned long long id = list[i / 81];
+    fix_walk(count, list, shards, seg_cap, blockIdx.y * gridDim.x + blockIdx.x, gridDim.x * gridDim.y, 81u,
+             [&](unsigned long long i, unsigned long long id) {
         const int k = (int)(i % 81);
         const unsigned wgs = (unsigned)(HVC_TILE * P.nw);
         const int lane = (int)(id % wgs);
         const unsigned long long t = id / wgs;
         const int tile = (int)(t % (unsigned)P.tiles_per_frame);
         const size_t f = (size_t)(t / (unsigned)P.tiles_per_frame);
-        if (f >= (size_t)P.n_frames) continue;
+        if (f >= (size_t)P.n_frames) return;
         const Ref444 rr = locate444(P, tile, lane, (int)wgs, HVC_444_TILE_BW * P.nw);
-        if (!rr.store || rr.p == 0) continue;
+        if (!rr.store || rr.p == 0) return;
         const int c = rr.bx * 8 - 1 + k % 9, r = rr.by * 8 - 1 + k / 9;
-        if (c < 0 || r < 0 || c >= aw || r >= ah) continue;
+        if (c < 0 || r < 0 || c >= aw || r >= ah) return;
         reinterp_sample(P.out + f * P.out_fs + P.pl[rr.p].out_off, W, aw, ah, c, r);
-    }
+    });
 }
 
 
@@ -1424,13 +1397,15 @@
     }();
     const int sel = P.kernel_sel ? P.kernel_sel : P.dc_plane ? 0 : env_sel;
     if (P.dc_plane && sel != 0) return hipErrorInvalidValue;
+    DecodeParams Q = P;
+    Q.fix_shards = FIX_SHARDS;
+    Q.fix_seg_cap = fix_seg_cap((unsigned long long)grid.x * grid.y, HVC_TILE);
     if (sel == 3)
-        hipLaunchKernelGGL(k_decode_q16, grid, dim3(HVC_TILE), 0, s, P);
+        hipLaunchKernelGGL(k_decode_q16, grid, dim3(HVC_TILE), 0, s, Q);
     else if (sel == 1)
-        hipLaunchKernelGGL(k_decode_fast, grid, dim3(HVC_TILE), 0, s, P);
+        hipLaunchKernelGGL(k_decode_fast, grid, dim3(HVC_TILE), 0, s, Q);
     else {
         static const unsigned pad = [] { const char *v = getenv("HVC_DEC_LDS_PAD"); return v ? (unsigned)atoi(v) : 0u; }();
-        DecodeParams Q = P;
         Q.xcd_map = xcd_map_for(grid.x, grid.y, Q.xcd_magic);
         if (P.dc_plane)
             hipLaunchKernelGGL(k_decode_packed<true>, grid, dim3(HVC_TILE), pad, s, Q);
@@ -1440,7 +1415,8 @@
     e = hipGetLastError();
     if (e != hipSuccess) return e;
     if (k1 && (e = hipEventRecord(k1, s)) != hipSuccess) return e;
-    hipLaunchKernelGGL(k_decode_wide, dim3(HVC_FIXUP_WGS), dim3(HVC_FIXUP_LANES), 0, s, P, P.fix_count, P.fix_list, (const long long *)nullptr);
+    hipLaunchKernelGGL(k_decode_wide, dim3(HVC_FIXUP_WGS), dim3(HVC_FIXUP_LANES), 0, s, Q, (const unsigned *)Q.fix_count,
+                       (const unsigned *)Q.fix_list, Q.fix_shards, Q.fix_seg_cap, (const long long *)nullptr);
     return hipGetLastError();
 }
 
@@ -1449,7 +1425,7 @@
     DecodeParams Q = P;
     Q.fix_count_next = nullptr;
     Q.wide_total = nullptr;
-    hipLaunchKernelGGL(k_decode_wide, dim3(64), dim3(64), 0, s, Q, count, ids, dcs);
+    hipLaunchKernelGGL(k_decode_wide, dim3(64), dim3(64), 0, s, Q, count, ids, 1u, 0u, dcs);
     return hipGetLastError();
 }
 
@@ -1458,7 +1434,7 @@
     Decode444Params Q = P;
     Q.fix_count_next = nullptr;
     Q.wide_total = nullptr;
-    hipLaunchKernelGGL(k_decode_wide_444, dim3(64), dim3(64), 0, s, Q, count, ids, 0ull, dcs);
+    hipLaunchKernelGGL(k_decode_wide_444, dim3(64), dim3(64), 0, s, Q, count, ids, 1u, 0u, 0ull, dcs);
     const size_t W = (size_t)P.width;
     const bool aligned = (W % 16 == 0) && (P.out_fs % 16 == 0) && ((uintptr_t)P.out % 16 == 0);
     const long long hw = aligned ? P.pl[1].aw / 8 : P.pl[1].aw;
@@ -1466,9 +1442,9 @@
     const long long want = seams > (long long)n_host * 81 ? seams : (long long)n_host * 81;
     const dim3 rgrid((unsigned)((want + 255) / 256) ? (unsigned)((want + 255) / 256) : 1u, (unsigned)P.n_frames, 1);
     if (aligned)
-        hipLaunchKernelGGL(k_reinterp_444<true>, rgrid, dim3(256), 0, s, Q, count, ids, 0);
+        hipLaunchKernelGGL(k_reinterp_444<true>, rgrid, dim3(256), 0, s, Q, count, ids, 1u, 0u, 0);
     else
-        hipLaunchKernelGGL(k_reinterp_444<false>, rgrid, dim3(256), 0, s, Q, count, ids, 0);
+        hipLaunchKernelGGL(k_reinterp_444<false>, rgrid, dim3(256), 0, s, Q, count, ids, 1u, 0u, 0);
     return hipGetLastError();
 }
 
@@ -1514,10 +1490,10 @@
         const unsigned long long total = (unsigned long long)P.n_frames * P.tiles_per_frame * HVC_TILE * P.nw;
         if (k0) (void)hipEventRecord(k0, s);
         hipLaunchKernelGGL(k_decode_wide_444, dim3(4096), dim3(64), 0, s, P, (const unsigned *)nullptr,
-                           (const unsigned *)nullptr, total, (const long long *)nullptr);
+                           (const unsigned *)nullptr, 1u, 0u, total, (const long long *)nullptr);
         if (k1) (void)hipEventRecord(k1, s);
         hipLaunchKernelGGL(k_reinterp_444<false>, dim3((unsigned)((2 * per_plane + 255) / 256), (unsigned)P.n_frames, 1),
-                           dim3(256), 0, s, P, (const unsigned *)P.fix_count, (const unsigned *)P.fix_list, 1);
+                           dim3(256), 0, s, P, (const unsigned *)P.fix_count, (const unsigned *)P.fix_list, 1u, 0u, 1);
         return hipGetLastError();
     }
     const size_t W = (size_t)P.width;
@@ -1527,6 +1503,8 @@
     Decode444Params Q = P;
     Q.skip = only;
     Q.xcd_map = xcd_map_for((unsigned)(P.tiles_per_frame - P.tile0), (unsigned)P.n_frames, Q.xcd_magic, true);
+    Q.fix_shards = FIX_SHARDS;
+    Q.fix_seg_cap = fix_seg_cap((unsigned long long)(P.tiles_per_frame - P.tile0) * (unsigned long long)P.n_frames, (unsigned)(HVC_TILE * P.nw));
     static const unsigned pad = [] { const char *v = getenv("HVC_444_LDS_PAD"); return v ? (unsigned)atoi(v) : 0u; }();
     if (!aligned && P.nw != 1) return hipErrorInvalidValue;
     const dim3 cgrid((unsigned)(P.tiles_per_frame - P.tile0), (unsigned)P.n_frames, 1);
@@ -1539,17 +1517,17 @@
     else
         launch_444_kernel<true, 4>(Q, cgrid, pad, s);
     if (k1) (void)hipEventRecord(k1, s);
-    hipLaunchKernelGGL(k_decode_wide_444, dim3(256), dim3(64), 0, s, P, (const unsigned *)P.fix_count,
-                       (const unsigned *)P.fix_list, 0ull, (const long long *)nullptr);
+    hipLaunchKernelGGL(k_decode_wide_444, dim3(256), dim3(64), 0, s, Q, (const unsigned *)Q.fix_count,
+                       (const unsigned *)Q.fix_list, Q.fix_shards, Q.fix_seg_cap, 0ull, (const long long *)nullptr);
     const long long hw = aligned ? P.pl[1].aw / 8 : P.pl[1].aw;
     const long long seams = 2 * (long long)(P.c_tiles_y - 1) * hw;
     const dim3 rgrid((unsigned)((seams + 255) / 256) ? (unsigned)((seams + 255) / 256) : 1u, (unsigned)P.n_frames, 1);
     if (aligned)
-        hipLaunchKernelGGL(k_reinterp_444<true>, rgrid, dim3(256), 0, s, P, (const unsigned *)P.fix_count,
-                           (const unsigned *)P.fix_list, 0);
+        hipLaunchKernelGGL(k_reinterp_444<true>, rgrid, dim3(256), 0, s, Q, (const unsigned *)Q.fix_count,
+                           (const unsigned *)Q.fix_list, Q.fix_shards, Q.fix_seg_cap, 0);
     else
-        hipLaunchKernelGGL(k_reinterp_444<false>, rgrid, dim3(256), 0, s, P, (const unsigned *)P.fix_count,
-                           (const unsigned *)P.fix_list, 0);
+        hipLaunchKernelGGL(k_reinterp_444<false>, rgrid, dim3(256), 0, s, Q, (const unsigned *)Q.fix_count,
+                           (const unsigned *)Q.fix_list, Q.fix_shards, Q.fix_seg_cap, 0);
     return hipGetLastError();
 }
 
diff --git a/video-coding_amd/csrc/hvc_mixed.h b/video-coding_amd/csrc/hvc_mixed.h
--- a/video-coding_amd/csrc/hvc_mixed.h
+++ b/video-coding_amd/csrc/hvc_mixed.h
@@ -20,7 +20,10 @@
     int wide_first;
     int xcd_map;
     unsigned xcd_magic;
+    unsigned fix_shards, fix_seg_cap;
 };
+
+size_t mixed_fix_list_entries(size_t n_units);
 
 hipError_t launch_decode_mixed(const MixedParams &P, hipStream_t s, hipEvent_t k0 = nullptr, hipEvent_t k1 = nullptr);
 
diff --git a/video-coding_amd/csrc/hvc_mixed.hip b/video-coding_amd/csrc/hvc_mixed.hip
--- a/video-coding_amd/csrc/hvc_mixed.hip
+++ b/video-coding_amd/csrc/hvc_mixed.hip
@@ -189,12 +189,7 @@
         flag = active && bad;
     }
     const unsigned long long m = __ballot(flag);
-    if (m) {
-        unsigned base = 0;
-        if (lane == 0) base = atomicAdd(P.fix_count, (unsigned)__popcll(m));
-        base = __shfl(base, 0);
-        if (flag) P.fix_list[base + (unsigned)__popcll(m & ((1ull << lane) - 1ull))] = unit * HVC_MIXED_UNIT + (unsigned)lane;
-    }
+    if (m) fix_append(P.fix_count, P.fix_list, P.fix_shards, P.fix_seg_cap, m, flag, lane, unit * HVC_MIXED_UNIT + (unsigned)lane);
 }
 
 template <bool COL>
@@ -275,20 +270,17 @@
 #define HVC_MIXED_WIDE_WGS 512
 #define HVC_MIXED_WIDE_LANES 256
 __global__ __launch_bounds__(HVC_MIXED_WIDE_LANES) void k_decode_mixed_wide(MixedParams P) {
-    const unsigned long long n = (unsigned long long)*P.fix_count;
-    if (blockIdx.x == 0 && threadIdx.x == 0) {
-        if (P.fix_count_next) *P.fix_count_next = 0;
-        if (P.wide_total) *P.wide_total = P.wide_first ? n : *P.wide_total + n;
-    }
-    for (unsigned long long i = (unsigned long long)blockIdx.x * blockDim.x + threadIdx.x; i < n;
-         i += (unsigned long long)gridDim.x * blockDim.x) {
-        const unsigned id = P.fix_list[i];
+    if (blockIdx.x == 0) {
+        const unsigned long long n = fix_total_and_clear(P.fix_count, P.fix_count_next, P.fix_shards);
+        if (threadIdx.x == 0 && P.wide_total) *P.wide_total = P.wide_first ? n : *P.wide_total + n;
+    }
+    fix_walk(P.fix_count, P.fix_list, P.fix_shards, P.fix_seg_cap, blockIdx.x, gridDim.x, 1u, [&](unsigned long long, unsigned id) {
         const unsigned unit = id / HVC_MIXED_UNIT, lane = id % HVC_MIXED_UNIT;
-        if (unit >= P.n_units) continue;
+        if (unit >= P.n_units) return;
         const MixedPlaneK K = P.planes[P.map[unit]];
-        if (unit < K.unit0) continue;
+        if (unit < K.unit0) return;
         const unsigned long long b = (unsigned long long)(unit - K.unit0) * HVC_MIXED_UNIT + lane;
-        if (b >= (unsigned long long)K.nblk) continue;
+        if (b >= (unsigned long long)K.nblk) return;
         const MixedRef br = mixed_block(P, K, (int)b);
         const uint4 *src = reinterpret_cast<const uint4 *>(br.coef);
         unsigned w[32], out[8][2];
@@ -303,9 +295,13 @@
         m_block_wide(w, P.tables[K.table].qt, out);
 #pragma unroll
         for (int j = 0; j < 8; j++) m_store_row(br.pix + (size_t)j * br.stride, out[j][0], out[j][1]);
-    }
-}
-
+    });
+}
+
+}
+
+size_t mixed_fix_list_entries(size_t n_units) {
+    return fix_list_entries((n_units + HVC_MIXED_GROUP - 1) / HVC_MIXED_GROUP, HVC_MIXED_LANES);
 }
 
 hipError_t launch_decode_mixed(const MixedParams &P, hipStream_t s, hipEvent_t k0, hipEvent_t k1) {
@@ -314,6 +310,8 @@
     const unsigned groups = (P.n_units + HVC_MIXED_GROUP - 1) / HVC_MIXED_GROUP;
     MixedParams Q = P;
     Q.xcd_map = xcd_map_for(groups, 1, Q.xcd_magic);
+    Q.fix_shards = FIX_SHARDS;
+    Q.fix_seg_cap = fix_seg_cap(groups, HVC_MIXED_LANES);
     if (k0 && (e = hipEventRecord(k0, s)) != hipSuccess) return e;
     hipLaunchKernelGGL(k_decode_mixed, dim3(groups), dim3(HVC_MIXED_LANES), 0, s, Q);
     if ((e = hipGetLastError()) != hipSuccess) return e;
```

Result: no change. 1.339 million (-0.8%).
